# ISU-PAAL/DeepDFA

Hardware: NVIDIA H100
Metric: CFG graphs/sec (train step) (higher is better)
Workload: dtype f32 (GRU GEMMs: bf16x3 split operands, f32 accumulate)

## Files before the change

deepdfa_b200/csrc/abi.cu:

```cuda
#include <stdarg.h>
#include <stdlib.h>
#include <string.h>

#include <atomic>

#include "common.cuh"

namespace ddfa {
static std::atomic<long long> g_launches{0};
void count_launch() { g_launches.fetch_add(1, std::memory_order_relaxed); }

static thread_local char g_err[512] = "";

static thread_local bool g_chain_break = true;
void chain_break() { g_chain_break = true; }
bool chain_take_break() {
  const bool b = g_chain_break;
  g_chain_break = false;
  return b;
}

static std::atomic<int> g_tuning[DDFA_TUNE__COUNT] = {
    {23},
    {15},
    {9},
    {0},
    {2},
    {0},
};
int l2_hints() { return g_tuning[DDFA_TUNE_L2_HINTS].load(std::memory_order_relaxed); }
int pdl_mask() { return g_tuning[DDFA_TUNE_PDL_MASK].load(std::memory_order_relaxed); }
int gather_variant() { return g_tuning[DDFA_TUNE_GATHER_VARIANT].load(std::memory_order_relaxed); }
int gate_bwd_tma() { return g_tuning[DDFA_TUNE_GATE_BWD_TMA].load(std::memory_order_relaxed); }
int gather_src_groups() { return g_tuning[DDFA_TUNE_GATHER_SRC_GROUPS].load(std::memory_order_relaxed); }

void set_error(const char *fmt, ...) {
  va_list ap;
  va_start(ap, fmt);
  vsnprintf(g_err, sizeof(g_err), fmt, ap);
  va_end(ap);
}
}

extern "C" {

int ddfa_abi_version(void) { return DDFA_ABI_VERSION; }

const char *ddfa_last_error(void) { return ddfa::g_err; }

int ddfa_engine_available(int engine) {
  if (engine == DDFA_ENGINE_SIMT) return 1;
  if (engine == DDFA_ENGINE_TCGEN05) return 1;
  return 0;
}

int ddfa_tuning_set(int key, int value) {
  DDFA_REQUIRE(key >= 0 && key < DDFA_TUNE__COUNT, "ddfa_tuning_set: unknown key %d", key);
  DDFA_REQUIRE(key != DDFA_TUNE_FWD_PAIR || value == 0, "ddfa_tuning_set: DDFA_TUNE_FWD_PAIR must be 0 (no CTA-pair forward kernel on sm_90a)");
  ddfa::g_tuning[key].store(value, std::memory_order_relaxed);
  return DDFA_OK;
}
int ddfa_tuning_get(int key) {
  if (key < 0 || key >= DDFA_TUNE__COUNT) return -1;
  return ddfa::g_tuning[key].load(std::memory_order_relaxed);
}

int ddfa_debug_set(int key, int value) {
  switch (key) {
    case 2: {
      int rc = ddfa::gru_tc3_trace_enable(value);
      return rc != DDFA_OK ? rc : ddfa::gru_tc2b_trace_enable(value);
    }
    default: ddfa::set_error("ddfa_debug_set: unknown key %d", key); return DDFA_ERR_INVALID_ARG;
  }
}

int ddfa_debug_read(int key, void *host_out, size_t bytes) {
  DDFA_REQUIRE(host_out != nullptr, "ddfa_debug_read: null output");
  switch (key) {
    case 2: return ddfa::gru_tc2b_trace_read(host_out, bytes);
    case 3: return ddfa::gru_tc3_trace_read(host_out, bytes);
    case 4: {
      DDFA_REQUIRE(bytes >= sizeof(int), "ddfa_debug_read: key 4 needs 4 bytes");
      const int v = ddfa::gather_tma_errors();
      memcpy(host_out, &v, sizeof(int));
      return DDFA_OK;
    }
    default: ddfa::set_error("ddfa_debug_read: unknown key %d", key); return DDFA_ERR_INVALID_ARG;
  }
}

long long ddfa_launch_count(void) { return ddfa::g_launches.load(std::memory_order_relaxed); }

int ddfa_device_supported(void) {
  int dev = 0;
  DDFA_CUDA(cudaGetDevice(&dev));
  int major = 0, minor = 0;
  DDFA_CUDA(cudaDeviceGetAttribute(&major, cudaDevAttrComputeCapabilityMajor, dev));
  DDFA_CUDA(cudaDeviceGetAttribute(&minor, cudaDevAttrComputeCapabilityMinor, dev));
  return (major == 9 && minor == 0) ? 1 : 0;
}

}
```

deepdfa_b200/csrc/common.cuh:

```cuda
#pragma once
#include <cuda_runtime.h>
#include <stdint.h>
#include <stdio.h>

#include "../../include/ddfa_b200.h"

namespace ddfa {

void set_error(const char *fmt, ...);
void count_launch();

inline cudaStream_t as_stream(void *s) { return reinterpret_cast<cudaStream_t>(s); }

#define DDFA_REQUIRE(cond, ...)            \
  do {                                     \
    if (!(cond)) {                         \
      ddfa::set_error(__VA_ARGS__);        \
      return DDFA_ERR_INVALID_ARG;         \
    }                                      \
  } while (0)

#define DDFA_CHECK_LAUNCH(name)                                                        \
  do {                                                                                 \
    cudaError_t e__ = cudaGetLastError();                                              \
    if (e__ != cudaSuccess) {                                                          \
      ddfa::set_error("%s: launch failed: %s", name, cudaGetErrorString(e__));         \
      return DDFA_ERR_CUDA;                                                            \
    }                                                                                  \
    ddfa::count_launch();                                                              \
  } while (0)

#define DDFA_CUDA(call)                                                                \
  do {                                                                                 \
    cudaError_t e__ = (call);                                                          \
    if (e__ != cudaSuccess) {                                                          \
      ddfa::set_error("%s failed: %s", #call, cudaGetErrorString(e__));                \
      return DDFA_ERR_CUDA;                                                            \
    }                                                                                  \
  } while (0)

__device__ __forceinline__ void pdl_launch_dependents() { asm volatile("griddepcontrol.launch_dependents;" ::: "memory"); }
__device__ __forceinline__ void pdl_wait() { asm volatile("griddepcontrol.wait;" ::: "memory"); }
int pdl_mask();
int gather_variant();
int gather_src_groups();
int gate_bwd_tma();
void chain_break();
bool chain_take_break();

template <typename... KArgs, typename... Args>
inline cudaError_t launch_chain_cluster(int which, int cluster_x, void (*kernel)(KArgs...), dim3 grid, dim3 block, size_t smem,
                                        cudaStream_t stream, Args... args) {
  cudaLaunchConfig_t cfg = {};
  cfg.gridDim = grid;
  cfg.blockDim = block;
  cfg.dynamicSmemBytes = smem;
  cfg.stream = stream;
  cudaLaunchAttribute attr[2];
  int n = 0;
  if (cluster_x > 1) {
    attr[n].id = cudaLaunchAttributeClusterDimension;
    attr[n].val.clusterDim.x = (unsigned)cluster_x;
    attr[n].val.clusterDim.y = 1;
    attr[n].val.clusterDim.z = 1;
    ++n;
  }
  const bool brk = chain_take_break();
  if ((pdl_mask() & which) && !brk) {
    attr[n].id = cudaLaunchAttributeProgrammaticStreamSerialization;
    attr[n].val.programmaticStreamSerializationAllowed = 1;
    ++n;
  }
  cfg.attrs = attr;
  cfg.numAttrs = n;
  return cudaLaunchKernelEx(&cfg, kernel, static_cast<KArgs>(args)...);
}
template <typename... KArgs, typename... Args>
inline cudaError_t launch_chain(int which, void (*kernel)(KArgs...), dim3 grid, dim3 block, size_t smem, cudaStream_t stream, Args... args) {
  return launch_chain_cluster(which, 1, kernel, grid, block, smem, stream, args...);
}

int adam_step_inc_launch(int32_t *step_count, cudaStream_t stream);

inline bool aligned16(const void *p) { return (reinterpret_cast<uintptr_t>(p) & 15u) == 0; }

constexpr int kNumSMs = 132;

int sgemm(int ta, int tb, int M, int N, int K, float alpha, const float *A, int lda, const float *B, int ldb,
          float beta, float *C, int ldc, int split_k, cudaStream_t stream);
size_t act_image_bytes(int64_t n);
int act_to_image(const float *x, int32_t N, void *image, cudaStream_t stream);
size_t gru_tc3_packed_bytes();
int gru_tc3_prepare(const float *w_fold, const float *b_fold, const float *b_ih, const float *w_hh, const float *b_hh, void *packed,
                    cudaStream_t stream);
int gru_tc3_step_fwd(const void *s_img, const void *h_img, const float *h, const int32_t *indptr, int32_t N, float *h_out,
                     void *h_out_img, float *save_gates, void *save_gates_packed, const void *packed, cudaStream_t stream);
int gru_tc3_trace_enable(int on);
int gru_tc3_trace_read(void *host, size_t bytes);
int gru_tc2b_trace_enable(int on);
int gru_tc2b_trace_read(void *host, size_t bytes);
size_t gru_tc2_workspace_bytes();
int gru_tc2_prepare(const float *w_fold, const float *b_fold, const float *b_ih, const float *w_hh, const float *b_hh,
                    void *workspace, size_t workspace_bytes, cudaStream_t stream);
int gru_tc2_step_fwd(const void *s_img, const void *h_img, const float *h, const int32_t *indptr, int32_t N, float *h_out,
                     void *h_out_img, float *save_gates, void *save_gates_packed, const void *workspace, size_t workspace_bytes,
                     cudaStream_t stream);
size_t gru_tc2_bwd_workspace_bytes(int32_t N, int32_t slots);
void *gru_tc2_bwd_s_image_scratch(void *workspace, int32_t N);
int gru_tc2_prepare_bwd(const float *w_fold, const float *w_hh, void *workspace, size_t workspace_bytes, cudaStream_t stream);
int gru_tc2_step_bwd(const float *dh_out, const float *ds_in, const int32_t *indptr_t, const int32_t *indices_t, const float *h,
                     const void *h_img_in, const void *s_img, const float *gates, const void *gates_packed, const int32_t *indptr, int32_t N, float *ds, float *dh, float *dw_fold, float *db_fold, float *db_ih,
                     float *dw_hh, float *db_hh, void *workspace, size_t workspace_bytes, int wgrad_mode, cudaStream_t stream);
int gru_tc2_bwd_finish(int32_t N, float *dw_fold, float *dw_hh, void *workspace, size_t workspace_bytes, cudaStream_t stream);
int gru_tc2_bwd_wgrad_batched(const void *const *s_imgs, const void *const *h_imgs, int32_t steps, int32_t N, float *dw_fold,
                              float *dw_hh, void *workspace, size_t workspace_bytes, cudaStream_t stream);

int launch_gather_tma(int variant, const int32_t *indptr, const int32_t *indices, const float *h, int32_t N, float *out, int accumulate,
                      cudaStream_t stream);
int gather_tma_errors();

__device__ __forceinline__ float4 ldg_nc_f4(const float *p) {
  float4 v;
  asm volatile("ld.global.nc.v4.f32 {%0,%1,%2,%3}, [%4];"
               : "=f"(v.x), "=f"(v.y), "=f"(v.z), "=f"(v.w)
               : "l"(p));
  return v;
}

__device__ __forceinline__ float4 ldg_cg_f4(const float *p) { return __ldcg(reinterpret_cast<const float4 *>(p)); }

__device__ __forceinline__ uint64_t l2_policy(int kind) {
  uint64_t p;
  if (kind == 1) asm volatile("createpolicy.fractional.L2::evict_first.b64 %0, 1.0;" : "=l"(p));
  else if (kind == 2) asm volatile("createpolicy.fractional.L2::evict_last.b64 %0, 1.0;" : "=l"(p));
  else asm volatile("createpolicy.fractional.L2::evict_normal.b64 %0, 1.0;" : "=l"(p));
  return p;
}
__device__ __forceinline__ void st_f32_hint(float *p, float v, uint64_t pol) {
  asm volatile("st.global.L2::cache_hint.f32 [%0], %1, %2;" ::"l"(p), "f"(v), "l"(pol) : "memory");
}
__device__ __forceinline__ void st_f4_hint(float *p, const float4 &v, uint64_t pol) {
  asm volatile("st.global.L2::cache_hint.v4.f32 [%0], {%1,%2,%3,%4}, %5;" ::"l"(p), "f"(v.x), "f"(v.y), "f"(v.z), "f"(v.w), "l"(pol) : "memory");
}
__device__ __forceinline__ void st_f2_hint(float *p, const float2 &v, uint64_t pol) {
  asm volatile("st.global.L2::cache_hint.v2.f32 [%0], {%1,%2}, %3;" ::"l"(p), "f"(v.x), "f"(v.y), "l"(pol) : "memory");
}
__device__ __forceinline__ void st_u4_hint(void *p, const uint4 &v, uint64_t pol) {
  asm volatile("st.global.L2::cache_hint.v4.u32 [%0], {%1,%2,%3,%4}, %5;" ::"l"(p), "r"(v.x), "r"(v.y), "r"(v.z), "r"(v.w), "l"(pol) : "memory");
}
__device__ __forceinline__ float4 ldg_cg_f4_hint(const float *p, uint64_t pol) {
  float4 v;
  asm volatile("ld.global.cg.L2::cache_hint.v4.f32 {%0,%1,%2,%3}, [%4], %5;" : "=f"(v.x), "=f"(v.y), "=f"(v.z), "=f"(v.w) : "l"(p), "l"(pol));
  return v;
}
__device__ __forceinline__ float ldg_cg_f32_hint(const float *p, uint64_t pol) {
  float v;
  asm volatile("ld.global.cg.L2::cache_hint.f32 %0, [%1], %2;" : "=f"(v) : "l"(p), "l"(pol));
  return v;
}
__device__ __forceinline__ void st_u32_hint(void *p, uint32_t v, uint64_t pol) {
  asm volatile("st.global.L2::cache_hint.u32 [%0], %1, %2;" ::"l"(p), "r"(v), "l"(pol) : "memory");
}
__device__ __forceinline__ void st_u2_hint(void *p, const uint2 &v, uint64_t pol) {
  asm volatile("st.global.L2::cache_hint.v2.u32 [%0], {%1,%2}, %3;" ::"l"(p), "r"(v.x), "r"(v.y), "l"(pol) : "memory");
}
__device__ __forceinline__ void st_f32_hint_if(bool pred, float *p, float v, uint64_t pol) {
  asm volatile("{\n.reg .pred q;\nsetp.ne.b32 q, %3, 0;\n@q st.global.L2::cache_hint.f32 [%0], %1, %2;\n}" ::"l"(p), "f"(v), "l"(pol), "r"((int)pred) : "memory");
}
__device__ __forceinline__ void st_u32_hint_if(bool pred, void *p, uint32_t v, uint64_t pol) {
  asm volatile("{\n.reg .pred q;\nsetp.ne.b32 q, %3, 0;\n@q st.global.L2::cache_hint.u32 [%0], %1, %2;\n}" ::"l"(p), "r"(v), "l"(pol), "r"((int)pred) : "memory");
}
__device__ __forceinline__ void st_u2_hint_if(bool pred, void *p, const uint2 &v, uint64_t pol) {
  asm volatile("{\n.reg .pred q;\nsetp.ne.b32 q, %4, 0;\n@q st.global.L2::cache_hint.v2.u32 [%0], {%1,%2}, %3;\n}" ::"l"(p), "r"(v.x), "r"(v.y), "l"(pol), "r"((int)pred)
               : "memory");
}
int l2_hints();

__device__ __forceinline__ float warp_sum(float v) {
#pragma unroll
  for (int o = 16; o > 0; o >>= 1) v += __shfl_xor_sync(0xffffffffu, v, o);
  return v;
}
__device__ __forceinline__ float warp_max(float v) {
#pragma unroll
  for (int o = 16; o > 0; o >>= 1) v = fmaxf(v, __shfl_xor_sync(0xffffffffu, v, o));
  return v;
}

__device__ __forceinline__ float sigmoidf_acc(float x) { return 1.0f / (1.0f + expf(-x)); }

__device__ __forceinline__ void f4_add(float4 &a, const float4 &b) {
  a.x += b.x; a.y += b.y; a.z += b.z; a.w += b.w;
}
__device__ __forceinline__ void f4_fma(float4 &a, float s, const float4 &b) {
  a.x = fmaf(s, b.x, a.x); a.y = fmaf(s, b.y, a.y); a.z = fmaf(s, b.z, a.z); a.w = fmaf(s, b.w, a.w);
}
__device__ __forceinline__ float f4_dot(const float4 &a, const float4 &b) {
  return a.x * b.x + a.y * b.y + a.z * b.z + a.w * b.w;
}

}
```

deepdfa_b200/csrc/gru_step.cu:

```cuda
#include "common.cuh"

namespace ddfa {

__global__ void __launch_bounds__(256) gru_gate_fwd_kernel(const float *__restrict__ gi_raw, const float *__restrict__ gh_raw,
                                                           const float *__restrict__ h, const int32_t *__restrict__ indptr,
                                                           const float *__restrict__ b_fold, const float *__restrict__ b_ih,
                                                           const float *__restrict__ b_hh, int32_t N, int32_t D,
                                                           float *__restrict__ h_out, float *__restrict__ gates) {
  const int dq = D >> 2;
  const int64_t t = blockIdx.x * (int64_t)blockDim.x + threadIdx.x;
  if (t >= (int64_t)N * dq) return;
  const int32_t n = (int32_t)(t / dq);
  const int c = (int)(t - (int64_t)n * dq) * 4;
  const float deg = (float)(indptr[n + 1] - indptr[n]);
  const float *gi = gi_raw + (int64_t)n * 3 * D;
  const float *gh = gh_raw + (int64_t)n * 3 * D;
  const float4 hv = *reinterpret_cast<const float4 *>(h + (int64_t)n * D + c);
  float4 g[3][2];
#pragma unroll
  for (int q = 0; q < 3; ++q) {
    const float4 a = *reinterpret_cast<const float4 *>(gi + q * D + c);
    const float4 bf = *reinterpret_cast<const float4 *>(b_fold + q * D + c);
    const float4 bi = *reinterpret_cast<const float4 *>(b_ih + q * D + c);
    g[q][0] = make_float4(fmaf(deg, bf.x, a.x) + bi.x, fmaf(deg, bf.y, a.y) + bi.y, fmaf(deg, bf.z, a.z) + bi.z,
                          fmaf(deg, bf.w, a.w) + bi.w);
    const float4 b = *reinterpret_cast<const float4 *>(gh + q * D + c);
    const float4 bh = *reinterpret_cast<const float4 *>(b_hh + q * D + c);
    g[q][1] = make_float4(b.x + bh.x, b.y + bh.y, b.z + bh.z, b.w + bh.w);
  }
  float4 r, z, nn, o;
#define GATE(f)                                            \
  r.f = sigmoidf_acc(g[0][0].f + g[0][1].f);               \
  z.f = sigmoidf_acc(g[1][0].f + g[1][1].f);               \
  nn.f = tanhf(fmaf(r.f, g[2][1].f, g[2][0].f));           \
  o.f = fmaf(z.f, hv.f - nn.f, nn.f);
  GATE(x) GATE(y) GATE(z) GATE(w)
#undef GATE
  *reinterpret_cast<float4 *>(h_out + (int64_t)n * D + c) = o;
  if (gates) {
    const int64_t plane = (int64_t)N * D, off = (int64_t)n * D + c;
    *reinterpret_cast<float4 *>(gates + off) = r;
    *reinterpret_cast<float4 *>(gates + plane + off) = z;
    *reinterpret_cast<float4 *>(gates + 2 * plane + off) = nn;
    *reinterpret_cast<float4 *>(gates + 3 * plane + off) = g[2][1];
  }
}

constexpr int kGateBwdRows = 128;
__global__ void __launch_bounds__(256) gru_gate_bwd_kernel(const float *__restrict__ dh_out, const float *__restrict__ h,
                                                           const float *__restrict__ gates, const int32_t *__restrict__ indptr,
                                                           int32_t N, int32_t D, float *__restrict__ dgi, float *__restrict__ dgh,
                                                           float *__restrict__ dh_part, float *__restrict__ db_fold,
                                                           float *__restrict__ db_ih, float *__restrict__ db_hh) {
  extern __shared__ float red[];
  const int c = threadIdx.x * 4;
  const int64_t plane = (int64_t)N * D;
  float4 acc[7];
#pragma unroll
  for (int i = 0; i < 7; ++i) acc[i] = make_float4(0.f, 0.f, 0.f, 0.f);
  const int32_t row0 = blockIdx.x * kGateBwdRows;
  const int32_t row1 = min(N, row0 + kGateBwdRows);
  for (int32_t n = row0 + threadIdx.y; n < row1; n += blockDim.y) {
    const int64_t off = (int64_t)n * D + c;
    const float deg = (float)(indptr[n + 1] - indptr[n]);
    const float4 d = *reinterpret_cast<const float4 *>(dh_out + off);
    const float4 hv = *reinterpret_cast<const float4 *>(h + off);
    const float4 r = *reinterpret_cast<const float4 *>(gates + off);
    const float4 z = *reinterpret_cast<const float4 *>(gates + plane + off);
    const float4 nn = *reinterpret_cast<const float4 *>(gates + 2 * plane + off);
    const float4 ghn = *reinterpret_cast<const float4 *>(gates + 3 * plane + off);
    float4 qr, qz, qn, qnr, dhp;
#define BWD(f)                                               \
  {                                                          \
    const float dz = d.f * (hv.f - nn.f);                    \
    const float dn = d.f * (1.f - z.f);                      \
    dhp.f = d.f * z.f;                                       \
    qn.f = dn * (1.f - nn.f * nn.f);                         \
    qz.f = dz * z.f * (1.f - z.f);                           \
    qr.f = qn.f * ghn.f * r.f * (1.f - r.f);                 \
    qnr.f = qn.f * r.f;                                      \
  }
    BWD(x) BWD(y) BWD(z) BWD(w)
#undef BWD
    float *gi = dgi + (int64_t)n * 3 * D + c;
    float *gh = dgh + (int64_t)n * 3 * D + c;
    *reinterpret_cast<float4 *>(gi) = qr;
    *reinterpret_cast<float4 *>(gi + D) = qz;
    *reinterpret_cast<float4 *>(gi + 2 * D) = qn;
    *reinterpret_cast<float4 *>(gh) = qr;
    *reinterpret_cast<float4 *>(gh + D) = qz;
    *reinterpret_cast<float4 *>(gh + 2 * D) = qnr;
    *reinterpret_cast<float4 *>(dh_part + off) = dhp;
    f4_add(acc[0], qr); f4_add(acc[1], qz); f4_add(acc[2], qn); f4_add(acc[3], qnr);
    f4_fma(acc[4], deg, qr); f4_fma(acc[5], deg, qz); f4_fma(acc[6], deg, qn);
  }
#pragma unroll
  for (int i = 0; i < 7; ++i) *reinterpret_cast<float4 *>(&red[((int64_t)threadIdx.y * 7 + i) * D + c]) = acc[i];
  __syncthreads();
  if (threadIdx.y == 0) {
#pragma unroll
    for (int i = 0; i < 7; ++i) {
      float4 sum = acc[i];
      for (int y = 1; y < blockDim.y; ++y) f4_add(sum, *reinterpret_cast<const float4 *>(&red[((int64_t)y * 7 + i) * D + c]));
      acc[i] = sum;
    }
#define RED4(ptr, v) atomicAdd((ptr) + 0, (v).x); atomicAdd((ptr) + 1, (v).y); atomicAdd((ptr) + 2, (v).z); atomicAdd((ptr) + 3, (v).w);
    RED4(db_ih + c, acc[0]) RED4(db_ih + D + c, acc[1]) RED4(db_ih + 2 * D + c, acc[2])
    RED4(db_hh + c, acc[0]) RED4(db_hh + D + c, acc[1]) RED4(db_hh + 2 * D + c, acc[3])
    RED4(db_fold + c, acc[4]) RED4(db_fold + D + c, acc[5]) RED4(db_fold + 2 * D + c, acc[6])
#undef RED4
  }
}

__global__ void fold_bias_kernel(const float *__restrict__ w_ih, const float *__restrict__ b, int32_t D, float *__restrict__ b_fold) {
  const int row = blockIdx.x * (blockDim.x >> 5) + (threadIdx.x >> 5);
  const int lane = threadIdx.x & 31;
  if (row >= 3 * D) return;
  float s = 0.f;
  for (int k = lane; k < D; k += 32) s = fmaf(w_ih[(int64_t)row * D + k], b[k], s);
  s = warp_sum(s);
  if (lane == 0) b_fold[row] = s;
}
__global__ void fold_bias_bwd_outer_kernel(const float *__restrict__ db_fold, const float *__restrict__ b, int32_t D, float *__restrict__ dw_ih) {
  const int64_t t = blockIdx.x * (int64_t)blockDim.x + threadIdx.x;
  if (t >= (int64_t)3 * D * D) return;
  const int j = (int)(t / D), k = (int)(t % D);
  dw_ih[t] = fmaf(db_fold[j], b[k], dw_ih[t]);
}
__global__ void __launch_bounds__(256) fold_bias_bwd_vec_kernel(const float *__restrict__ w_ih, const float *__restrict__ db_fold,
                                                                int32_t D, float *__restrict__ db) {
  __shared__ float red[8][33];
  const int k = blockIdx.x * 32 + threadIdx.x;
  float s = 0.f;
  if (k < D)
    for (int j = threadIdx.y; j < 3 * D; j += 8) s = fmaf(w_ih[(int64_t)j * D + k], db_fold[j], s);
  red[threadIdx.y][threadIdx.x] = s;
  __syncthreads();
  if (threadIdx.y == 0 && k < D) {
    float t = 0.f;
#pragma unroll
    for (int y = 0; y < 8; ++y) t += red[y][threadIdx.x];
    db[k] += t;
  }
}

}

extern "C" {

int ddfa_fold_weights_fwd(const float *w_msg, const float *b_msg, const float *w_ih, int32_t D, float *w_fold,
                          float *b_fold, void *stream_) {
  using namespace ddfa;
  DDFA_REQUIRE(D > 0 && D % 4 == 0, "ddfa_fold_weights_fwd: D=%d must be a positive multiple of 4", D);
  DDFA_REQUIRE(w_msg && b_msg && w_ih && w_fold && b_fold, "ddfa_fold_weights_fwd: NULL pointer");
  cudaStream_t stream = as_stream(stream_);
  int rc = sgemm(0, 0, 3 * D, D, D, 1.f, w_ih, D, w_msg, D, 0.f, w_fold, D, 1, stream);
  if (rc) return rc;
  fold_bias_kernel<<<(3 * D + 7) / 8, 256, 0, stream>>>(w_ih, b_msg, D, b_fold);
  DDFA_CHECK_LAUNCH("fold_bias_kernel");
  return DDFA_OK;
}

int ddfa_fold_weights_bwd(const float *w_msg, const float *b_msg, const float *w_ih, const float *dw_fold,
                          const float *db_fold, int32_t D, float *dw_msg, float *db_msg, float *dw_ih, void *stream_) {
  using namespace ddfa;
  DDFA_REQUIRE(D > 0 && D % 4 == 0, "ddfa_fold_weights_bwd: D=%d must be a positive multiple of 4", D);
  DDFA_REQUIRE(w_msg && b_msg && w_ih && dw_fold && db_fold && dw_msg && db_msg && dw_ih, "ddfa_fold_weights_bwd: NULL pointer");
  cudaStream_t stream = as_stream(stream_);
  int rc = sgemm(0, 1, 3 * D, D, D, 1.f, dw_fold, D, w_msg, D, 1.f, dw_ih, D, 1, stream);
  if (rc) return rc;
  rc = sgemm(1, 0, D, D, 3 * D, 1.f, w_ih, D, dw_fold, D, 1.f, dw_msg, D, 1, stream);
  if (rc) return rc;
  const int64_t tot = (int64_t)3 * D * D;
  fold_bias_bwd_outer_kernel<<<(unsigned)((tot + 255) / 256), 256, 0, stream>>>(db_fold, b_msg, D, dw_ih);
  DDFA_CHECK_LAUNCH("fold_bias_bwd_outer_kernel");
  fold_bias_bwd_vec_kernel<<<(D + 31) / 32, dim3(32, 8), 0, stream>>>(w_ih, db_fold, D, db_msg);
  DDFA_CHECK_LAUNCH("fold_bias_bwd_vec_kernel");
  return DDFA_OK;
}

size_t ddfa_gru_step_workspace_bytes(int32_t N, int32_t D, int engine) {
  if (N < 0 || D <= 0) return 0;
  if (engine == DDFA_ENGINE_TCGEN05) return D == 128 ? ddfa::gru_tc2_workspace_bytes() + 2 * ddfa::act_image_bytes(N) : 16;
  return sizeof(float) * 2 * (size_t)N * 3 * (size_t)D;
}

size_t ddfa_act_image_bytes(int64_t num_nodes) { return num_nodes < 0 ? 0 : ddfa::act_image_bytes(num_nodes); }

int ddfa_act_to_image(const float *x, int32_t N, int32_t D, void *image, void *stream_) {
  using namespace ddfa;
  DDFA_REQUIRE(N >= 0 && D == 128, "ddfa_act_to_image: activation images exist for D == 128 only (N=%d D=%d)", N, D);
  if (N == 0) return DDFA_OK;
  DDFA_REQUIRE(x && image && aligned16(x) && aligned16(image), "ddfa_act_to_image: NULL or unaligned pointer");
  return act_to_image(x, N, image, as_stream(stream_));
}

int ddfa_gru_step_fwd_image(const void *s_image, const void *h_image, const float *h, const int32_t *indptr, int32_t N,
                            int32_t D, float *h_out, void *h_out_image, float *save_gates, const void *workspace,
                            size_t workspace_bytes, void *stream_) {
  using namespace ddfa;
  DDFA_REQUIRE(N >= 0 && D == 128, "ddfa_gru_step_fwd_image: the tcgen05 engine supports D == 128 only (N=%d D=%d)", N, D);
  if (N == 0) return DDFA_OK;
  DDFA_REQUIRE(s_image && h_image && h && indptr && h_out, "ddfa_gru_step_fwd_image: NULL pointer");
  return gru_tc2_step_fwd(s_image, h_image, h, indptr, N, h_out, h_out_image, save_gates, nullptr, workspace, workspace_bytes,
                          as_stream(stream_));
}

size_t ddfa_gru_gates_packed_bytes(int32_t N, int32_t D) { return (N < 0 || D <= 0) ? 0 : (size_t)N * (size_t)D * 8; }

int ddfa_gru_step_fwd_image_v2(const void *s_image, const void *h_image, const float *h, const int32_t *indptr, int32_t N, int32_t D,
                               float *h_out, void *h_out_image, void *save_gates_packed, const void *workspace, size_t workspace_bytes,
                               void *stream_) {
  using namespace ddfa;
  DDFA_REQUIRE(N >= 0 && D == 128, "ddfa_gru_step_fwd_image_v2: the tcgen05 engine supports D == 128 only (N=%d D=%d)", N, D);
  if (N == 0) return DDFA_OK;
  DDFA_REQUIRE(s_image && h_image && indptr, "ddfa_gru_step_fwd_image_v2: NULL pointer");
  DDFA_REQUIRE(h_out || h_out_image, "ddfa_gru_step_fwd_image_v2: neither h_out nor h_out_image given");
  return gru_tc2_step_fwd(s_image, h_image, h, indptr, N, h_out, h_out_image, nullptr, save_gates_packed, workspace, workspace_bytes,
                          as_stream(stream_));
}

static int check_step_args(const char *who, int32_t N, int32_t D, int engine) {
  using namespace ddfa;
  DDFA_REQUIRE(N >= 0 && D > 0 && D % 4 == 0 && D <= 1024, "%s: unsupported shape N=%d D=%d", who, N, D);
  DDFA_REQUIRE(engine == DDFA_ENGINE_SIMT || engine == DDFA_ENGINE_TCGEN05, "%s: unknown engine %d", who, engine);
  if (engine == DDFA_ENGINE_TCGEN05 && D != 128) {
    set_error("%s: the tcgen05 engine supports D == 128 only (got %d); select DDFA_ENGINE_SIMT", who, D);
    return DDFA_ERR_UNSUPPORTED;
  }
  return DDFA_OK;
}

int ddfa_gru_step_prepare(const float *w_fold, const float *b_fold, const float *b_ih, const float *w_hh, const float *b_hh,
                          int32_t D, int engine, void *workspace, size_t workspace_bytes, void *stream_) {
  using namespace ddfa;
  int rc = check_step_args("ddfa_gru_step_prepare", 0, D, engine);
  if (rc) return rc;
  if (engine == DDFA_ENGINE_SIMT) return DDFA_OK;
  DDFA_REQUIRE(w_fold && b_fold && b_ih && w_hh && b_hh, "ddfa_gru_step_prepare: NULL pointer");
  return gru_tc2_prepare(w_fold, b_fold, b_ih, w_hh, b_hh, workspace, workspace_bytes, as_stream(stream_));
}

int ddfa_gru_step_fwd(const float *s, const float *h, const int32_t *indptr, const float *w_fold, const float *b_fold,
                      const float *b_ih, const float *w_hh, const float *b_hh, int32_t N, int32_t D, float *h_out,
                      float *save_gates, void *workspace, size_t workspace_bytes, int engine, void *stream_) {
  using namespace ddfa;
  int rc = check_step_args("ddfa_gru_step_fwd", N, D, engine);
  if (rc) return rc;
  if (N == 0) return DDFA_OK;
  DDFA_REQUIRE(s && h && indptr && w_fold && b_fold && b_ih && w_hh && b_hh && h_out, "ddfa_gru_step_fwd: NULL pointer");
  cudaStream_t stream = as_stream(stream_);
  if (workspace_bytes < ddfa_gru_step_workspace_bytes(N, D, engine) || workspace == nullptr) {
    set_error("ddfa_gru_step_fwd: workspace too small (%zu < %zu)", workspace_bytes, ddfa_gru_step_workspace_bytes(N, D, engine));
    return DDFA_ERR_WORKSPACE;
  }
  if (engine == DDFA_ENGINE_TCGEN05) {
    uint8_t *ws8 = static_cast<uint8_t *>(workspace);
    void *s_img = ws8 + gru_tc2_workspace_bytes();
    void *h_img = ws8 + gru_tc2_workspace_bytes() + act_image_bytes(N);
    rc = act_to_image(s, N, s_img, stream);
    if (rc) return rc;
    rc = act_to_image(h, N, h_img, stream);
    if (rc) return rc;
    return gru_tc2_step_fwd(s_img, h_img, h, indptr, N, h_out, nullptr, save_gates, nullptr, workspace, workspace_bytes, stream);
  }
  float *gi = static_cast<float *>(workspace);
  float *gh = gi + (size_t)N * 3 * D;
  rc = sgemm(0, 1, N, 3 * D, D, 1.f, s, D, w_fold, D, 0.f, gi, 3 * D, 1, stream);
  if (rc) return rc;
  rc = sgemm(0, 1, N, 3 * D, D, 1.f, h, D, w_hh, D, 0.f, gh, 3 * D, 1, stream);
  if (rc) return rc;
  const int64_t tot = (int64_t)N * (D / 4);
  gru_gate_fwd_kernel<<<(unsigned)((tot + 255) / 256), 256, 0, stream>>>(gi, gh, h, indptr, b_fold, b_ih, b_hh, N, D, h_out, save_gates);
  DDFA_CHECK_LAUNCH("gru_gate_fwd_kernel");
  return DDFA_OK;
}

size_t ddfa_gru_step_bwd_workspace_bytes(int32_t N, int32_t D, int engine) {
  if (N < 0 || D <= 0) return 0;
  return ddfa_gru_step_bwd_workspace_bytes_steps(N, D, engine, 1);
}

size_t ddfa_gru_step_bwd_workspace_bytes_steps(int32_t N, int32_t D, int engine, int32_t steps) {
  if (N < 0 || D <= 0) return 0;
  if (engine == DDFA_ENGINE_TCGEN05) return D == 128 ? ddfa::gru_tc2_bwd_workspace_bytes(N, steps) : 16;
  return sizeof(float) * 2 * (size_t)N * 3 * (size_t)D;
}

int ddfa_gru_bwd_wgrad_batched(const void *const *s_images, const void *const *h_images, int32_t steps, int32_t N, int32_t D,
                               float *dw_fold, float *dw_hh, void *workspace, size_t workspace_bytes, void *stream_) {
  using namespace ddfa;
  DDFA_REQUIRE(N >= 0 && D == 128, "ddfa_gru_bwd_wgrad_batched: the tcgen05 engine supports D == 128 only (N=%d D=%d)", N, D);
  DDFA_REQUIRE(s_images && h_images && dw_fold && dw_hh, "ddfa_gru_bwd_wgrad_batched: NULL pointer");
  if (N == 0) return DDFA_OK;
  return gru_tc2_bwd_wgrad_batched(s_images, h_images, steps, N, dw_fold, dw_hh, workspace, workspace_bytes, as_stream(stream_));
}

int ddfa_gru_step_bwd_image(const float *dh_out, const float *ds_prev, const int32_t *indptr_t, const int32_t *indices_t,
                            const float *h, const void *h_image, const void *s_image, const float *gates,
                            const int32_t *indptr, int32_t N, int32_t D, float *ds, float *dh, float *dw_fold, float *db_fold,
                            float *db_ih, float *dw_hh, float *db_hh, void *workspace, size_t workspace_bytes, int wgrad_mode,
                            void *stream_) {
  using namespace ddfa;
  DDFA_REQUIRE(N >= 0 && D == 128, "ddfa_gru_step_bwd_image: the tcgen05 engine supports D == 128 only (N=%d D=%d)", N, D);
  DDFA_REQUIRE((wgrad_mode >= 0 && wgrad_mode <= 2) || (wgrad_mode >= 16 && wgrad_mode < 32),
               "ddfa_gru_step_bwd_image: wgrad_mode must be 0, 1, 2 or DDFA_WGRAD_KEEP(slot < 16) (got %d)", wgrad_mode);
  if (N == 0) return DDFA_OK;
  DDFA_REQUIRE(dh_out && h && s_image && gates && indptr && ds && dh && dw_fold && db_fold && db_ih && dw_hh && db_hh,
               "ddfa_gru_step_bwd_image: NULL pointer");
  DDFA_REQUIRE(dh != dh_out, "ddfa_gru_step_bwd_image: dh must not alias dh_out");
  DDFA_REQUIRE(ds_prev == nullptr || (indptr_t && indices_t), "ddfa_gru_step_bwd_image: ds_prev given without the transposed CSR");
  DDFA_REQUIRE(ds_prev == nullptr || ds_prev != ds, "ddfa_gru_step_bwd_image: ds must not alias ds_prev");
  return gru_tc2_step_bwd(dh_out, ds_prev, indptr_t, indices_t, h, h_image, s_image, gates, nullptr, indptr, N, ds, dh, dw_fold, db_fold, db_ih, dw_hh, db_hh, workspace,
                          workspace_bytes, wgrad_mode, as_stream(stream_));
}

int ddfa_gru_step_bwd_image_v2(const float *dh_out, const float *ds_prev, const int32_t *indptr_t, const int32_t *indices_t,
                               const float *h, const void *h_image, const void *s_image, const void *gates_packed,
                               const int32_t *indptr, int32_t N, int32_t D, float *ds, float *dh, float *dw_fold, float *db_fold,
                               float *db_ih, float *dw_hh, float *db_hh, void *workspace, size_t workspace_bytes, int wgrad_mode,
                               void *stream_) {
  using namespace ddfa;
  DDFA_REQUIRE(N >= 0 && D == 128, "ddfa_gru_step_bwd_image_v2: the tcgen05 engine supports D == 128 only (N=%d D=%d)", N, D);
  DDFA_REQUIRE((wgrad_mode >= 0 && wgrad_mode <= 2) || (wgrad_mode >= 16 && wgrad_mode < 32),
               "ddfa_gru_step_bwd_image_v2: wgrad_mode must be 0, 1, 2 or DDFA_WGRAD_KEEP(slot < 16) (got %d)", wgrad_mode);
  if (N == 0) return DDFA_OK;
  DDFA_REQUIRE(dh_out && h_image && s_image && gates_packed && indptr && ds && dh && dw_fold && db_fold && db_ih && dw_hh && db_hh,
               "ddfa_gru_step_bwd_image_v2: NULL pointer");
  DDFA_REQUIRE(dh != dh_out, "ddfa_gru_step_bwd_image_v2: dh must not alias dh_out");
  DDFA_REQUIRE(ds_prev == nullptr || (indptr_t && indices_t), "ddfa_gru_step_bwd_image_v2: ds_prev given without the transposed CSR");
  DDFA_REQUIRE(ds_prev == nullptr || ds_prev != ds, "ddfa_gru_step_bwd_image_v2: ds must not alias ds_prev");
  return gru_tc2_step_bwd(dh_out, ds_prev, indptr_t, indices_t, h, h_image, s_image, nullptr, gates_packed, indptr, N, ds, dh, dw_fold, db_fold,
                          db_ih, dw_hh, db_hh, workspace, workspace_bytes, wgrad_mode, as_stream(stream_));
}

int ddfa_gru_step_bwd_finish(int32_t N, int32_t D, float *dw_fold, float *dw_hh, void *workspace, size_t workspace_bytes,
                             void *stream_) {
  using namespace ddfa;
  DDFA_REQUIRE(N >= 0 && D == 128 && dw_fold && dw_hh, "ddfa_gru_step_bwd_finish: bad arguments (N=%d D=%d)", N, D);
  if (N == 0) return DDFA_OK;
  return gru_tc2_bwd_finish(N, dw_fold, dw_hh, workspace, workspace_bytes, as_stream(stream_));
}

int ddfa_gru_step_prepare_bwd(const float *w_fold, const float *w_hh, int32_t D, int engine, void *workspace,
                              size_t workspace_bytes, void *stream_) {
  using namespace ddfa;
  int rc = check_step_args("ddfa_gru_step_prepare_bwd", 0, D, engine);
  if (rc) return rc;
  if (engine == DDFA_ENGINE_SIMT) return DDFA_OK;
  DDFA_REQUIRE(w_fold && w_hh, "ddfa_gru_step_prepare_bwd: NULL pointer");
  return gru_tc2_prepare_bwd(w_fold, w_hh, workspace, workspace_bytes, as_stream(stream_));
}

int ddfa_gru_step_bwd(const float *dh_out, const float *h, const float *s, const float *gates, const int32_t *indptr,
                      const float *w_fold, const float *w_hh, int32_t N, int32_t D, float *ds, float *dh,
                      float *dw_fold, float *db_fold, float *db_ih, float *dw_hh, float *db_hh, void *workspace,
                      size_t workspace_bytes, int engine, void *stream_) {
  using namespace ddfa;
  int rc = check_step_args("ddfa_gru_step_bwd", N, D, engine);
  if (rc) return rc;
  if (N == 0) return DDFA_OK;
  DDFA_REQUIRE(dh_out && h && s && gates && indptr && w_fold && w_hh && ds && dh && dw_fold && db_fold && db_ih && dw_hh && db_hh,
               "ddfa_gru_step_bwd: NULL pointer");
  DDFA_REQUIRE(dh != dh_out, "ddfa_gru_step_bwd: dh must not alias dh_out");
  cudaStream_t stream = as_stream(stream_);
  const size_t need = ddfa_gru_step_bwd_workspace_bytes(N, D, engine);
  if (workspace_bytes < need || workspace == nullptr) {
    set_error("ddfa_gru_step_bwd: workspace too small (%zu < %zu)", workspace_bytes, need);
    return DDFA_ERR_WORKSPACE;
  }
  if (engine == DDFA_ENGINE_TCGEN05) {
    void *s_img = gru_tc2_bwd_s_image_scratch(workspace, N);
    rc = act_to_image(s, N, s_img, stream);
    if (rc) return rc;
    return gru_tc2_step_bwd(dh_out, nullptr, nullptr, nullptr, h, nullptr, s_img, gates, nullptr, indptr, N, ds, dh, dw_fold, db_fold, db_ih, dw_hh, db_hh,
                            workspace, workspace_bytes, 0, stream);
  }
  float *dgi = static_cast<float *>(workspace);
  float *dgh = dgi + (size_t)N * 3 * D;
  dim3 block(D / 4, 256 / (D / 4) > 0 ? 256 / (D / 4) : 1);
  const size_t smem = sizeof(float) * block.y * 7 * D;
  gru_gate_bwd_kernel<<<(N + kGateBwdRows - 1) / kGateBwdRows, block, smem, stream>>>(dh_out, h, gates, indptr, N, D, dgi, dgh, dh,
                                                                                     db_fold, db_ih, db_hh);
  DDFA_CHECK_LAUNCH("gru_gate_bwd_kernel");
  rc = sgemm(0, 0, N, D, 3 * D, 1.f, dgi, 3 * D, w_fold, D, 0.f, ds, D, 1, stream);
  if (rc) return rc;
  rc = sgemm(0, 0, N, D, 3 * D, 1.f, dgh, 3 * D, w_hh, D, 1.f, dh, D, 1, stream);
  if (rc) return rc;
  const int tiles = ((3 * D + 127) / 128) * ((D + 127) / 128);
  int split = (2 * kNumSMs + tiles - 1) / tiles;
  const int k_tiles = (N + 15) / 16;
  if (split > k_tiles / 8) split = k_tiles / 8 > 0 ? k_tiles / 8 : 1;
  rc = sgemm(1, 0, 3 * D, D, N, 1.f, dgi, 3 * D, s, D, 1.f, dw_fold, D, split, stream);
  if (rc) return rc;
  rc = sgemm(1, 0, 3 * D, D, N, 1.f, dgh, 3 * D, h, D, 1.f, dw_hh, D, split, stream);
  return rc;
}

}
```

deepdfa_b200/csrc/gru_tc_bwd.cu:

```cuda
#include <cuda_fp16.h>

#include "tc_common.cuh"

namespace ddfa {
namespace tc2b {
using namespace tcc;

constexpr int kThreads = 320, kEpiWarps = 8;

constexpr int kGbWarps = 8;
struct GbRow {
  float4 d, hv, rr, zz, nn, gh;
  float deg;
  int tb, te;
};
__device__ __forceinline__ float4 bf16x4_to_f4(const uint2 &p) {
  return make_float4(__uint_as_float(p.x << 16), __uint_as_float(p.x & 0xffff0000u), __uint_as_float(p.y << 16), __uint_as_float(p.y & 0xffff0000u));
}
__device__ __forceinline__ void gb_load(GbRow &x, const float *__restrict__ dh_out, const float *__restrict__ h,
                                        const uint8_t *__restrict__ h_img_src, const float *__restrict__ gates,
                                        const uint4 *__restrict__ gates_packed, const int32_t *__restrict__ indptr,
                                        const int32_t *__restrict__ indptr_t, size_t plane, int64_t node, int col, bool ok,
                                        uint64_t pol_saved, uint64_t pol_dh) {
  x.tb = x.te = 0;
  if (ok) {
    if (indptr_t) { x.tb = __ldcg(indptr_t + node); x.te = __ldcg(indptr_t + node + 1); }
    const size_t off = (size_t)node * kD + col;
    x.d = ldg_cg_f4_hint(dh_out + off, pol_dh);
    uint2 hh = make_uint2(0u, 0u), hl = hh;
    uint4 g0 = make_uint4(0u, 0u, 0u, 0u), g1 = g0;
    if (h) x.hv = ldg_cg_f4_hint(h + off, pol_saved);
    else {
      hh = __ldcg(reinterpret_cast<const uint2 *>(h_img_src + image_offset(node, col, 0)));
      hl = __ldcg(reinterpret_cast<const uint2 *>(h_img_src + image_offset(node, col, 1)));
    }
    if (gates) {
      x.rr = ldg_cg_f4_hint(gates + off, pol_saved);
      x.zz = ldg_cg_f4_hint(gates + plane + off, pol_saved);
      x.nn = ldg_cg_f4_hint(gates + 2 * plane + off, pol_saved);
      x.gh = ldg_cg_f4_hint(gates + 3 * plane + off, pol_saved);
    } else {
      g0 = __ldcg(gates_packed + (off >> 1));
      g1 = __ldcg(gates_packed + (off >> 1) + 1);
    }
    x.deg = (float)(__ldcg(indptr + node + 1) - __ldcg(indptr + node));
    if (!h) {
      const float4 a = bf16x4_to_f4(hh), b = bf16x4_to_f4(hl);
      x.hv = make_float4(a.x + b.x, a.y + b.y, a.z + b.z, a.w + b.w);
    }
    if (!gates) {
      unpack_gates(make_uint2(g0.x, g0.y), x.rr.x, x.zz.x, x.nn.x, x.gh.x);
      unpack_gates(make_uint2(g0.z, g0.w), x.rr.y, x.zz.y, x.nn.y, x.gh.y);
      unpack_gates(make_uint2(g1.x, g1.y), x.rr.z, x.zz.z, x.nn.z, x.gh.z);
      unpack_gates(make_uint2(g1.z, g1.w), x.rr.w, x.zz.w, x.nn.w, x.gh.w);
    }
  }
}

__global__ void __launch_bounds__(32 * kGbWarps, 2) gate_bwd_image_kernel(const float *__restrict__ dh_out, const float *__restrict__ h,
                                                                          const uint8_t *__restrict__ h_img_src,
                                                                          const float *__restrict__ gates, const uint4 *__restrict__ gates_packed,
                                                                          const int32_t *__restrict__ indptr,
                                                                          const float *__restrict__ ds_in, const int32_t *__restrict__ indptr_t,
                                                                          const int32_t *__restrict__ indices_t,
                                                                          int32_t N, uint8_t *__restrict__ q_img, size_t img_stride,
                                                                          uint8_t *__restrict__ h_img, float *__restrict__ dhz,
                                                                          float *__restrict__ db_fold,
                                                                          float *__restrict__ db_ih, float *__restrict__ db_hh, int hints) {
  __shared__ float red[kGbWarps][7 * kD];
  const int lane = threadIdx.x & 31, warp = threadIdx.x >> 5;
  const int col = lane * 4;
  pdl_launch_dependents();
  pdl_wait();
  const uint64_t pol_saved = l2_policy((hints & 2) ? 1 : 0), pol_tmp = l2_policy((hints & 4) ? 2 : 0), pol_dh = l2_policy((hints & 8) ? 1 : 0);
  const size_t plane = (size_t)N * kD;
  float4 sum[7];
#pragma unroll
  for (int i = 0; i < 7; ++i) sum[i] = make_float4(0.f, 0.f, 0.f, 0.f);
  const int64_t Npad = ((int64_t)N + kTileM - 1) / kTileM * kTileM;
  const int64_t stride = (int64_t)gridDim.x * kGbWarps;

  auto finish = [&](const GbRow &x, int64_t node, bool ok) {
    float4 qr = make_float4(0.f, 0.f, 0.f, 0.f), qz = qr, qn = qr, qnr = qr, hv = qr;
    if (ok) {
      hv = x.hv;
      st_f4_hint(dhz + (size_t)node * kD + col, make_float4(x.d.x * x.zz.x, x.d.y * x.zz.y, x.d.z * x.zz.z, x.d.w * x.zz.w), pol_tmp);
#define BWDQ(f)                                                      \
  {                                                                  \
    const float dz_ = x.d.f * (x.hv.f - x.nn.f);                     \
    const float dn_ = x.d.f * (1.f - x.zz.f);                        \
    qn.f = dn_ * (1.f - x.nn.f * x.nn.f);                            \
    qz.f = dz_ * x.zz.f * (1.f - x.zz.f);                            \
    qr.f = qn.f * x.gh.f * x.rr.f * (1.f - x.rr.f);                  \
    qnr.f = qn.f * x.rr.f;                                           \
  }
      BWDQ(x) BWDQ(y) BWDQ(z) BWDQ(w)
#undef BWDQ
      f4_add(sum[0], qr); f4_add(sum[1], qz); f4_add(sum[2], qn); f4_add(sum[3], qnr);
      f4_fma(sum[4], x.deg, qr); f4_fma(sum[5], x.deg, qz); f4_fma(sum[6], x.deg, qn);
    }
    const size_t o_hi = image_offset(node, col, 0), o_lo = image_offset(node, col, 1);
    uint2 ph, pl;
    split4(qr, ph, pl);  *reinterpret_cast<uint2 *>(q_img + 0 * img_stride + o_hi) = ph; *reinterpret_cast<uint2 *>(q_img + 0 * img_stride + o_lo) = pl;
    split4(qz, ph, pl);  *reinterpret_cast<uint2 *>(q_img + 1 * img_stride + o_hi) = ph; *reinterpret_cast<uint2 *>(q_img + 1 * img_stride + o_lo) = pl;
    split4(qn, ph, pl);  *reinterpret_cast<uint2 *>(q_img + 2 * img_stride + o_hi) = ph; *reinterpret_cast<uint2 *>(q_img + 2 * img_stride + o_lo) = pl;
    split4(qnr, ph, pl); *reinterpret_cast<uint2 *>(q_img + 3 * img_stride + o_hi) = ph; *reinterpret_cast<uint2 *>(q_img + 3 * img_stride + o_lo) = pl;
    if (h_img) {
      split4(hv, ph, pl); *reinterpret_cast<uint2 *>(h_img + o_hi) = ph; *reinterpret_cast<uint2 *>(h_img + o_lo) = pl;
    }
  };

  for (int64_t node = (int64_t)blockIdx.x * kGbWarps + warp; node < Npad; node += 2 * stride) {
    const int64_t node2 = node + stride;
    GbRow a, b;
    const bool ok_a = node < N, ok_b = node2 < N;
    gb_load(a, dh_out, h, h_img_src, gates, gates_packed, indptr, indptr_t, plane, node, col, ok_a, pol_saved, pol_dh);
    gb_load(b, dh_out, h, h_img_src, gates, gates_packed, indptr, indptr_t, plane, node2, col, ok_b, pol_saved, pol_dh);
    if (indptr_t) {
      int ia[4], ib[4];
#pragma unroll
      for (int k = 0; k < 4; ++k) {
        ia[k] = (a.tb + k < a.te) ? __ldcg(indices_t + a.tb + k) : -1;
        ib[k] = (b.tb + k < b.te) ? __ldcg(indices_t + b.tb + k) : -1;
      }
      float4 va[4], vb[4];
#pragma unroll
      for (int k = 0; k < 4; ++k) {
        va[k] = ia[k] >= 0 ? ldg_cg_f4(ds_in + (size_t)ia[k] * kD + col) : make_float4(0.f, 0.f, 0.f, 0.f);
        vb[k] = ib[k] >= 0 ? ldg_cg_f4(ds_in + (size_t)ib[k] * kD + col) : make_float4(0.f, 0.f, 0.f, 0.f);
      }
#pragma unroll
      for (int k = 0; k < 4; ++k) { f4_add(a.d, va[k]); f4_add(b.d, vb[k]); }
      for (int j = a.tb + 4; j < a.te; ++j) f4_add(a.d, ldg_cg_f4(ds_in + (size_t)__ldcg(indices_t + j) * kD + col));
      for (int j = b.tb + 4; j < b.te; ++j) f4_add(b.d, ldg_cg_f4(ds_in + (size_t)__ldcg(indices_t + j) * kD + col));
    }
    finish(a, node, ok_a);
    if (node2 < Npad) finish(b, node2, ok_b);
  }
#pragma unroll
  for (int i = 0; i < 7; ++i) *reinterpret_cast<float4 *>(&red[warp][i * kD + col]) = sum[i];
  __syncthreads();
  for (int i = threadIdx.x; i < 7 * kD; i += 32 * kGbWarps) {
    float v_ = 0.f;
#pragma unroll
    for (int w = 0; w < kGbWarps; ++w) v_ += red[w][i];
    const int which = i >> 7, c_ = i & 127;
    if (which == 0) { atomicAdd(db_ih + c_, v_); atomicAdd(db_hh + c_, v_); }
    else if (which == 1) { atomicAdd(db_ih + kD + c_, v_); atomicAdd(db_hh + kD + c_, v_); }
    else if (which == 2) atomicAdd(db_ih + 2 * kD + c_, v_);
    else if (which == 3) atomicAdd(db_hh + 2 * kD + c_, v_);
    else atomicAdd(db_fold + (which - 4) * kD + c_, v_);
  }
}

constexpr int kGtRows = 32, kGtStages = 3, kGtConsumers = 16, kGtPre = 2;
constexpr int kGtOffD = 0, kGtOffG = kGtRows * kD * 4, kGtOffH = kGtOffG + kGtRows * kD * 8;
constexpr int kGtStageBytes = kGtOffH + kGtRows * kD * 4;
constexpr int kGtOffBar = kGtStages * kGtStageBytes;
constexpr int kGtSmem = kGtOffBar + 2 * kGtStages * 8 + 16;
constexpr int kGtThreads = 32 * kGtConsumers;

template <bool HF32, bool CSRP>
__global__ void __launch_bounds__(kGtThreads, 1) gate_bwd_tma_kernel(const float *__restrict__ dh_out, const float *__restrict__ h,
                                                                     const uint8_t *__restrict__ h_img_src, const uint2 *__restrict__ gates_packed,
                                                                     const int32_t *__restrict__ indptr, const float *__restrict__ ds_in,
                                                                     const int32_t *__restrict__ indptr_t, const int32_t *__restrict__ indices_t,
                                                                     int32_t N, uint8_t *__restrict__ q_img, size_t img_stride,
                                                                     float *__restrict__ dhz, float *__restrict__ db_fold, float *__restrict__ db_ih,
                                                                     float *__restrict__ db_hh, int hints) {
  extern __shared__ __align__(1024) uint8_t smem[];
  const uint32_t sbase = smem_u32(smem);
  const uint32_t bar0 = sbase + kGtOffBar;
  auto full = [&](int i) { return bar0 + 8u * i; };
  auto empty = [&](int i) { return bar0 + 8u * (kGtStages + i); };
  const int lane = threadIdx.x & 31, warp = threadIdx.x >> 5;
  const int64_t Npad = ((int64_t)N + kTileM - 1) / kTileM * kTileM;
  const int num_blocks = (int)(Npad / kGtRows);
  const int my_blocks = (num_blocks > (int)blockIdx.x) ? (num_blocks - 1 - (int)blockIdx.x) / (int)gridDim.x + 1 : 0;
  if (threadIdx.x == 0) {
    for (int i = 0; i < kGtStages; ++i) { mbar_init(full(i), 1); mbar_init(empty(i), kGtConsumers); }
    mbar_fence_init();
  }
  __syncthreads();
  pdl_launch_dependents();
  pdl_wait();
  float4 sum[7];
#pragma unroll
  for (int i = 0; i < 7; ++i) sum[i] = make_float4(0.f, 0.f, 0.f, 0.f);

  auto fill = [&](int k) {
    const uint64_t pol_saved = l2_policy((hints & 2) ? 1 : 0), pol_dh = l2_policy((hints & 8) ? 1 : 0);
    const int stage = k % kGtStages;
    const int64_t r0 = (int64_t)(blockIdx.x + (int64_t)k * gridDim.x) * kGtRows;
    const int valid = (int)max((int64_t)0, min((int64_t)kGtRows, (int64_t)N - r0));
    const uint32_t dst = sbase + stage * kGtStageBytes;
    const uint32_t bytes = (uint32_t)valid * (kD * 4 + kD * 8) + (HF32 ? (uint32_t)valid * kD * 4 : (uint32_t)kGtRows * kD * 4);
    mbar_arrive_expect_tx(full(stage), bytes);
    if (valid > 0) {
      bulk_g2s_hint(dst + kGtOffD, dh_out + r0 * kD, (uint32_t)valid * kD * 4, full(stage), pol_dh);
      bulk_g2s_hint(dst + kGtOffG, gates_packed + r0 * kD, (uint32_t)valid * kD * 8, full(stage), pol_saved);
    }
    if (HF32) {
      if (valid > 0) bulk_g2s_hint(dst + kGtOffH, h + r0 * kD, (uint32_t)valid * kD * 4, full(stage), pol_saved);
    } else {
      const uint8_t *tile = h_img_src + (size_t)(r0 >> 7) * kImageTileBytes + (size_t)(r0 & 127) * 128;
#pragma unroll
      for (int ch = 0; ch < 4; ++ch) bulk_g2s_hint(dst + kGtOffH + ch * (kGtRows * 128), tile + (size_t)ch * kChunkBytes, kGtRows * 128, full(stage), pol_saved);
    }
  };
  if (warp == 0 && elect_one())
    for (int k = 0; k < kGtStages && k < my_blocks; ++k) fill(k);
  __syncwarp();
  {
    const int col = lane * 4;
    const uint64_t pol_tmp = l2_policy((hints & 4) ? 2 : 0);
    static_assert(kGtPre == 2, "lane slots below assume two prefetched neighbours per row");
    auto load_scalars = [&](int kk) -> int {
      int v = 0;
      if (kk < my_blocks && lane < 8) {
        const int64_t nd = (int64_t)(blockIdx.x + (int64_t)kk * gridDim.x) * kGtRows + warp + 16 * ((lane >> 1) & 1);
        const int32_t *base = lane < 4 ? indptr : indptr_t;
        if (nd < N && base) v = __ldcg(base + nd + (lane & 1));
      }
      return v;
    };
    auto load_ids = [&](int sc) -> int {
      const int r_ = (lane >> 1) & 1, q_ = lane & 1;
      const int tb_ = __shfl_sync(0xffffffffu, sc, 4 + 2 * r_), te_ = __shfl_sync(0xffffffffu, sc, 5 + 2 * r_);
      int v = -1;
      if (lane >= 8 && lane < 12 && tb_ + q_ < te_) v = __ldcg(indices_t + tb_ + q_);
      return v;
    };
    int sc_cur = 0, sc_next = 0, id_cur = -1;
    if constexpr (CSRP) {
      sc_cur = load_scalars(0); sc_next = load_scalars(1);
      id_cur = load_ids(sc_cur);
    }
    for (int k = 0; k < my_blocks; ++k) {
      const int stage = k % kGtStages, use = k / kGtStages;
      const int64_t r0 = (int64_t)(blockIdx.x + (int64_t)k * gridDim.x) * kGtRows;
      int64_t node[2];
      bool ok[2];
      int tb[2], te[2], ip0[2], ip1[2];
      int id[2][kGtPre];
      if constexpr (CSRP) {
        const int sc_next2 = load_scalars(k + 2);
        const int id_next = load_ids(sc_next);
#pragma unroll
        for (int r = 0; r < 2; ++r) {
          node[r] = r0 + warp + 16 * r;
          ok[r] = node[r] < N;
          ip0[r] = __shfl_sync(0xffffffffu, sc_cur, 2 * r); ip1[r] = __shfl_sync(0xffffffffu, sc_cur, 2 * r + 1);
          tb[r] = __shfl_sync(0xffffffffu, sc_cur, 4 + 2 * r); te[r] = __shfl_sync(0xffffffffu, sc_cur, 5 + 2 * r);
#pragma unroll
          for (int q = 0; q < kGtPre; ++q) id[r][q] = __shfl_sync(0xffffffffu, id_cur, 8 + 2 * r + q);
        }
        sc_cur = sc_next; sc_next = sc_next2; id_cur = id_next;
      } else {
#pragma unroll
        for (int r = 0; r < 2; ++r) {
          node[r] = r0 + warp + 16 * r;
          ok[r] = node[r] < N;
          tb[r] = te[r] = ip0[r] = ip1[r] = 0;
          if (ok[r]) {
            ip0[r] = __ldcg(indptr + node[r]); ip1[r] = __ldcg(indptr + node[r] + 1);
            if (indptr_t) { tb[r] = __ldcg(indptr_t + node[r]); te[r] = __ldcg(indptr_t + node[r] + 1); }
          }
        }
#pragma unroll
        for (int r = 0; r < 2; ++r)
#pragma unroll
          for (int q = 0; q < kGtPre; ++q) id[r][q] = (tb[r] + q < te[r]) ? __ldcg(indices_t + tb[r] + q) : -1;
      }
      float4 gv[2][kGtPre];
#pragma unroll
      for (int r = 0; r < 2; ++r)
#pragma unroll
        for (int q = 0; q < kGtPre; ++q) gv[r][q] = id[r][q] >= 0 ? ldg_cg_f4(ds_in + (size_t)id[r][q] * kD + col) : make_float4(0.f, 0.f, 0.f, 0.f);
      mbar_wait(full(stage), use & 1);
      const uint8_t *st = smem + stage * kGtStageBytes;
#pragma unroll
      for (int r = 0; r < 2; ++r) {
        const int row = warp + 16 * r;
        float4 d = make_float4(0.f, 0.f, 0.f, 0.f), hv = d, rr = d, zz = d, nn = d, gh = d;
        if (ok[r]) {
          d = *reinterpret_cast<const float4 *>(st + kGtOffD + row * (kD * 4) + col * 4);
          const uint4 g0 = *reinterpret_cast<const uint4 *>(st + kGtOffG + row * (kD * 8) + col * 8);
          const uint4 g1 = *reinterpret_cast<const uint4 *>(st + kGtOffG + row * (kD * 8) + col * 8 + 16);
          unpack_gates(make_uint2(g0.x, g0.y), rr.x, zz.x, nn.x, gh.x);
          unpack_gates(make_uint2(g0.z, g0.w), rr.y, zz.y, nn.y, gh.y);
          unpack_gates(make_uint2(g1.x, g1.y), rr.z, zz.z, nn.z, gh.z);
          unpack_gates(make_uint2(g1.z, g1.w), rr.w, zz.w, nn.w, gh.w);
          if (HF32) {
            hv = *reinterpret_cast<const float4 *>(st + kGtOffH + row * (kD * 4) + col * 4);
          } else {
            const uint32_t off = (uint32_t)((col >> 6) * (kGtRows * 128) + row * 128 + (((((col & 63) >> 3) ^ (row & 7)) & 7) << 4) + (col & 7) * 2);
            const uint2 hh = *reinterpret_cast<const uint2 *>(st + kGtOffH + off);
            const uint2 hl = *reinterpret_cast<const uint2 *>(st + kGtOffH + 2 * (kGtRows * 128) + off);
            const float4 a = bf16x4_to_f4(hh), b = bf16x4_to_f4(hl);
            hv = make_float4(a.x + b.x, a.y + b.y, a.z + b.z, a.w + b.w);
          }
#pragma unroll
          for (int q = 0; q < kGtPre; ++q) f4_add(d, gv[r][q]);
          for (int j = tb[r] + kGtPre; j < te[r]; ++j) f4_add(d, ldg_cg_f4(ds_in + (size_t)__ldcg(indices_t + j) * kD + col));
        }
        float4 qr = make_float4(0.f, 0.f, 0.f, 0.f), qz = qr, qn = qr, qnr = qr;
        if (ok[r]) {
          const float deg = (float)(ip1[r] - ip0[r]);
          st_f4_hint(dhz + (size_t)node[r] * kD + col, make_float4(d.x * zz.x, d.y * zz.y, d.z * zz.z, d.w * zz.w), pol_tmp);
#define BWDQ2(f)                                         \
  {                                                      \
    const float dz_ = d.f * (hv.f - nn.f);               \
    const float dn_ = d.f * (1.f - zz.f);                \
    qn.f = dn_ * (1.f - nn.f * nn.f);                    \
    qz.f = dz_ * zz.f * (1.f - zz.f);                    \
    qr.f = qn.f * gh.f * rr.f * (1.f - rr.f);            \
    qnr.f = qn.f * rr.f;                                 \
  }
          BWDQ2(x) BWDQ2(y) BWDQ2(z) BWDQ2(w)
#undef BWDQ2
          f4_add(sum[0], qr); f4_add(sum[1], qz); f4_add(sum[2], qn); f4_add(sum[3], qnr);
          f4_fma(sum[4], deg, qr); f4_fma(sum[5], deg, qz); f4_fma(sum[6], deg, qn);
        }
        if (node[r] < Npad) {
          const size_t o_hi = image_offset(node[r], col, 0), o_lo = image_offset(node[r], col, 1);
          uint2 ph, pl;
          split4(qr, ph, pl);  *reinterpret_cast<uint2 *>(q_img + 0 * img_stride + o_hi) = ph; *reinterpret_cast<uint2 *>(q_img + 0 * img_stride + o_lo) = pl;
          split4(qz, ph, pl);  *reinterpret_cast<uint2 *>(q_img + 1 * img_stride + o_hi) = ph; *reinterpret_cast<uint2 *>(q_img + 1 * img_stride + o_lo) = pl;
          split4(qn, ph, pl);  *reinterpret_cast<uint2 *>(q_img + 2 * img_stride + o_hi) = ph; *reinterpret_cast<uint2 *>(q_img + 2 * img_stride + o_lo) = pl;
          split4(qnr, ph, pl); *reinterpret_cast<uint2 *>(q_img + 3 * img_stride + o_hi) = ph; *reinterpret_cast<uint2 *>(q_img + 3 * img_stride + o_lo) = pl;
        }
      }
      __syncwarp();
      if (lane == 0) mbar_arrive(empty(stage));
      if (warp == 0 && k + kGtStages < my_blocks) {
        if (elect_one()) {
          mbar_wait(empty(stage), use & 1);
          fill(k + kGtStages);
        }
        __syncwarp();
      }
    }
  }
  __syncthreads();
  float *red = reinterpret_cast<float *>(smem);
  {
#pragma unroll
    for (int i = 0; i < 7; ++i) *reinterpret_cast<float4 *>(&red[(warp * 7 + i) * kD + lane * 4]) = sum[i];
  }
  __syncthreads();
  for (int i = threadIdx.x; i < 7 * kD; i += kGtThreads) {
    float v_ = 0.f;
#pragma unroll
    for (int w = 0; w < kGtConsumers; ++w) v_ += red[(w * 7) * kD + i];
    const int which = i >> 7, c_ = i & 127;
    if (which == 0) { atomicAdd(db_ih + c_, v_); atomicAdd(db_hh + c_, v_); }
    else if (which == 1) { atomicAdd(db_ih + kD + c_, v_); atomicAdd(db_hh + kD + c_, v_); }
    else if (which == 2) atomicAdd(db_ih + 2 * kD + c_, v_);
    else if (which == 3) atomicAdd(db_hh + 2 * kD + c_, v_);
    else atomicAdd(db_fold + (which - 4) * kD + c_, v_);
  }
}

constexpr int kD3Stages = 2;
constexpr int kD3StageBytes = kImageTileBytes;
constexpr int kD3WChunkBytes = 64 * 128;
constexpr int kD3WBytes = 12 * kD3WChunkBytes;
constexpr int kD3OffStage = kD3WBytes;
constexpr int kD3OffBar = kD3OffStage + kD3Stages * kD3StageBytes;
constexpr int kD3SmemAlloc = kD3OffBar + (2 * kD3Stages + 1) * 8 + 1024;
constexpr int kD3Threads = 32 * kEpiWarps + 32;
constexpr size_t kD3PackedBytes = (size_t)4 * kD3WBytes;
static_assert(kD3SmemAlloc <= 232448, "shared memory budget");

__global__ void dgrad3_pack_kernel(const float *__restrict__ w_fold, const float *__restrict__ w_hh, uint8_t *__restrict__ packed) {
  const int idx = blockIdx.x * blockDim.x + threadIdx.x;
  if (idx >= 4 * 3 * 64 * 16) return;
  const int u = idx % 16, n = (idx / 16) % 64, g = (idx / (16 * 64)) % 3, rh = idx / (16 * 64 * 3);
  const int role = rh >> 1, half = rh & 1, kb = u >> 3;
  const float *W = role == 0 ? w_fold : w_hh;
  float x[8];
#pragma unroll
  for (int i = 0; i < 8; ++i) x[i] = W[(size_t)(g * kD + u * 8 + i) * kD + half * 64 + n];
  uint4 ph, pl;
  split8(x, ph, pl);
  uint8_t *base = packed + (size_t)rh * kD3WBytes + sw128_offset(n, (u & 7) * 8);
  *reinterpret_cast<uint4 *>(base + ((g * 2 + 0) * 2 + kb) * kD3WChunkBytes) = ph;
  *reinterpret_cast<uint4 *>(base + ((g * 2 + 1) * 2 + kb) * kD3WChunkBytes) = pl;
}

__global__ void __launch_bounds__(kD3Threads, 1) dgrad3_kernel(const uint8_t *__restrict__ q_img, size_t img_stride,
                                                               const float *__restrict__ dhz, const uint8_t *__restrict__ packed3,
                                                               int32_t N, float *__restrict__ ds, float *__restrict__ dh, int hints) {
  extern __shared__ uint8_t smem_raw[];
  uint8_t *smem = reinterpret_cast<uint8_t *>((reinterpret_cast<uintptr_t>(smem_raw) + 1023) & ~(uintptr_t)1023);
  const uint32_t sbase = smem_u32(smem);
  const uint32_t bar0 = sbase + kD3OffBar;
  auto full = [&](int i) { return bar0 + 8u * i; };
  auto empty = [&](int i) { return bar0 + 8u * (kD3Stages + i); };
  const uint32_t w_full = bar0 + 8u * (2 * kD3Stages);
  const int tron = (g_trace_on == 1);

  const int warp = threadIdx.x >> 5, lane = threadIdx.x & 31;
  const int rh = blockIdx.x & 3, role = rh >> 1, half = rh & 1;
  const int group = blockIdx.x >> 2, num_groups = gridDim.x >> 2;
  const int num_tiles = (N + kTileM - 1) / kTileM;
  const int my_tiles = (num_tiles > group) ? (num_tiles - 1 - group) / num_groups + 1 : 0;

  if (threadIdx.x == 0) {
    for (int i = 0; i < kD3Stages; ++i) { mbar_init(full(i), 1); mbar_init(empty(i), kEpiWarps); }
    mbar_init(w_full, 1);
    mbar_fence_init();
  }
  __syncthreads();
  if (threadIdx.x == 0) trace_stamp(tron, 0, 0);
  pdl_launch_dependents();

  if (warp == kEpiWarps) {
    if (my_tiles > 0 && elect_one()) {
      mbar_arrive_expect_tx(w_full, kD3WBytes);
      bulk_g2s(sbase, packed3 + (size_t)rh * kD3WBytes, kD3WBytes, w_full);
      pdl_wait();
      const uint64_t pol_q = l2_policy((hints & 64) ? 1 : 0);
      int cc = 0;
      for (int k = 0; k < my_tiles; ++k) {
        const int tile = num_tiles - 1 - (group + k * num_groups);
        for (int g = 0; g < 3; ++g, ++cc) {
          const int m = g < 2 ? g : (role == 0 ? 2 : 3);
          const int stage = cc % kD3Stages, use = cc / kD3Stages;
          if (use > 0) mbar_wait_bounded(empty(stage), (use - 1) & 1);
          mbar_arrive_expect_tx(full(stage), kD3StageBytes);
          bulk_g2s_hint(sbase + kD3OffStage + stage * kD3StageBytes, q_img + (size_t)m * img_stride + (size_t)tile * kImageTileBytes,
                        kD3StageBytes, full(stage), pol_q);
          if (g != 1) trace_stamp(tron, k, g == 0 ? 1 : 2);
        }
      }
    }
    return;
  }

  pdl_wait();
  if (my_tiles == 0) return;
  const int wg = warp >> 2;
  const int row0 = wg * 64 + (warp & 3) * 16 + (lane >> 2);
  const int col0 = half * 64 + 2 * (lane & 3);
  float *out = role == 0 ? ds : dh;
  const uint64_t pol_tmp = l2_policy((hints & 4) ? 2 : 0);
  const uint64_t pol_dhz = l2_policy((hints & 8) ? 1 : 0);
  mbar_wait_bounded(w_full, 0);
  const bool tr = (warp == 0 && lane == 0);
  int cc = 0, pending = -1;
  for (int k = 0; k < my_tiles; ++k) {
    const int tile = num_tiles - 1 - (group + k * num_groups);
    float acc[32];
    if (tr) { trace_stamp(tron, k, 7); trace_stamp(tron, k, 3); }
    for (int g = 0; g < 3; ++g, ++cc) {
      const int stage = cc % kD3Stages, use = cc / kD3Stages;
      mbar_wait_bounded(full(stage), use & 1);
      if (tr && g != 1) trace_stamp(tron, k, g == 0 ? 4 : 5);
      wgmma_fence();
      const uint32_t a0 = sbase + kD3OffStage + stage * kD3StageBytes + wg * 8192;
      const uint32_t w0 = sbase + g * 4 * kD3WChunkBytes;
#pragma unroll
      for (int kb = 0; kb < 2; ++kb) {
#pragma unroll
        for (int k4 = 0; k4 < 4; ++k4) {
          const uint64_t a_hi = gmma_desc(a0 + kb * kChunkBytes + k4 * 32), a_lo = gmma_desc(a0 + (2 + kb) * kChunkBytes + k4 * 32);
          const uint64_t b_hi = gmma_desc(w0 + kb * kD3WChunkBytes + k4 * 32), b_lo = gmma_desc(w0 + (2 + kb) * kD3WChunkBytes + k4 * 32);
          wgmma_n64<0, 0>(acc, a_hi, b_hi, (g == 0 && kb == 0 && k4 == 0) ? 0u : 1u);
          wgmma_n64<0, 0>(acc, a_hi, b_lo, 1u);
          wgmma_n64<0, 0>(acc, a_lo, b_hi, 1u);
        }
      }
      wgmma_commit();
      wgmma_wait<1>();
      __syncwarp();
      if (pending >= 0 && lane == 0) mbar_arrive(empty(pending));
      pending = stage;
    }
    float2 dv[2][8];
#pragma unroll
    for (int hh = 0; hh < 2; ++hh) {
      const int64_t node = (int64_t)tile * kTileM + row0 + 8 * hh;
#pragma unroll
      for (int j = 0; j < 8; ++j) {
        dv[hh][j] = make_float2(0.f, 0.f);
        if (role == 1 && node < N) {
          const float *p = dhz + node * kD + col0 + 8 * j;
          dv[hh][j] = make_float2(ldg_cg_f32_hint(p, pol_dhz), ldg_cg_f32_hint(p + 1, pol_dhz));
        }
      }
    }
    wgmma_wait<0>();
    wgmma_fence_regs(acc);
    if (tr) { trace_stamp(tron, k, 6); trace_stamp(tron, k, 8); }
    __syncwarp();
    if (lane == 0) mbar_arrive(empty(pending));
    pending = -1;
    if (tr) trace_stamp(tron, k, 9);
#pragma unroll
    for (int hh = 0; hh < 2; ++hh) {
      const int64_t node = (int64_t)tile * kTileM + row0 + 8 * hh;
      if (node < N) {
#pragma unroll
        for (int j = 0; j < 8; ++j)
          st_f2_hint(out + node * kD + col0 + 8 * j, make_float2(acc[4 * j + 2 * hh] + dv[hh][j].x, acc[4 * j + 2 * hh + 1] + dv[hh][j].y), pol_tmp);
      }
    }
    if (tr) trace_stamp(tron, k, 10);
  }
}

constexpr int kWgSlotBytes = kImageTileBytes;
constexpr int kWgSlots = 3;
constexpr int kWgOffBar = kWgSlots * kWgSlotBytes;
constexpr int kWgSmemAlloc = kWgOffBar + 2 * kWgSlots * 8 + 1024;
constexpr int kWgThreads = 32 * kEpiWarps + 32;
constexpr size_t kWgPartialFloats = (size_t)3 * kD * kD;
constexpr int kWgMaxSteps = 16;
struct WgBatch {
  const uint8_t *s_img[kWgMaxSteps];
  const uint8_t *h_img[kWgMaxSteps];
  int32_t steps;
};
__global__ void __launch_bounds__(kWgThreads, 1) wgrad_kernel(const uint8_t *__restrict__ q_img, size_t img_stride, size_t step_stride,
                                                              const __grid_constant__ WgBatch batch,
                                                              int32_t N, float *__restrict__ partial, int first, int hints) {
  extern __shared__ uint8_t smem_raw[];
  uint8_t *smem = reinterpret_cast<uint8_t *>((reinterpret_cast<uintptr_t>(smem_raw) + 1023) & ~(uintptr_t)1023);
  const uint32_t sbase = smem_u32(smem);
  const uint32_t bar0 = sbase + kWgOffBar;
  auto full = [&](int i) { return bar0 + 8u * i; };
  auto empty = [&](int i) { return bar0 + 8u * (kWgSlots + i); };

  const int warp = threadIdx.x >> 5, lane = threadIdx.x & 31;
  const int role = blockIdx.y / 3, g = blockIdx.y % 3;
  const int qm = g < 2 ? g : (role == 0 ? 2 : 3);
  const int num_tiles = (N + kTileM - 1) / kTileM;
  const int all_tiles = num_tiles * batch.steps;
  const int my_tiles = (all_tiles > (int)blockIdx.x) ? (all_tiles - 1 - (int)blockIdx.x) / (int)gridDim.x + 1 : 0;

  if (threadIdx.x == 0) {
    for (int i = 0; i < kWgSlots; ++i) { mbar_init(full(i), 1); mbar_init(empty(i), kEpiWarps); }
    mbar_fence_init();
  }
  __syncthreads();
  const int tron = (g_trace_on == 2) && blockIdx.y == 0;
  if (threadIdx.x == 0) trace_stamp(tron, 0, 0);

  if (warp == kEpiWarps) {
    if (elect_one()) {
      const uint64_t pol_wg = l2_policy((hints & 32) ? 1 : 0);
      for (int i = 0; i < my_tiles; ++i) {
        const int idx = (int)blockIdx.x + i * (int)gridDim.x;
        const int t = idx / num_tiles, tile = idx - t * num_tiles;
        for (int w = 0; w < 2; ++w) {
          const int cc = 2 * i + w, slot = cc % kWgSlots, use = cc / kWgSlots;
          if (use > 0) mbar_wait_bounded(empty(slot), (use - 1) & 1);
          const uint8_t *src = w == 0 ? (role == 0 ? batch.s_img[t] : batch.h_img[t]) : q_img + (size_t)t * step_stride + (size_t)qm * img_stride;
          mbar_arrive_expect_tx(full(slot), kWgSlotBytes);
          bulk_g2s_hint(sbase + slot * kWgSlotBytes, src + (size_t)tile * kImageTileBytes, kWgSlotBytes, full(slot), pol_wg);
          trace_stamp(tron, i, 1 + w);
        }
      }
    }
    return;
  }

  const int wg = warp >> 2;
  float acc[64], sum[64];
#pragma unroll
  for (int i = 0; i < 64; ++i) acc[i] = sum[i] = 0.f;
  for (int i = 0; i < my_tiles; ++i) {
    const int cb = 2 * i, ca = 2 * i + 1;
    mbar_wait_bounded(full(cb % kWgSlots), (cb / kWgSlots) & 1);
    if (warp == 0 && lane == 0) trace_stamp(tron, i, 3);
    mbar_wait_bounded(full(ca % kWgSlots), (ca / kWgSlots) & 1);
    if (warp == 0 && lane == 0) { trace_stamp(tron, i, 4); trace_stamp(tron, i, 5); }
    const uint32_t b0 = sbase + (cb % kWgSlots) * kWgSlotBytes;
    const uint32_t a0 = sbase + (ca % kWgSlots) * kWgSlotBytes + wg * kChunkBytes;
    constexpr uint32_t vs = 2 * kChunkBytes;
    wgmma_fence();
#pragma unroll
    for (int k16 = 0; k16 < kTileM / 16; ++k16) {
      const uint32_t koff = (uint32_t)k16 * 2048u;
      const uint64_t a_hi = gmma_desc(a0 + koff, kChunkBytes), a_lo = gmma_desc(a0 + vs + koff, kChunkBytes);
      const uint64_t b_hi = gmma_desc(b0 + koff, kChunkBytes), b_lo = gmma_desc(b0 + vs + koff, kChunkBytes);
      wgmma_n128<1, 1>(acc, a_hi, b_hi, k16 == 0 ? 0u : 1u);
      wgmma_n128<1, 1>(acc, a_lo, b_hi, 1u);
      wgmma_n128<1, 1>(acc, a_hi, b_lo, 1u);
    }
    wgmma_commit();
    if (warp == 0 && lane == 0) trace_stamp(tron, i, 6);
    wgmma_wait<0>();
    wgmma_fence_regs(acc);
    __syncwarp();
    if (lane == 0) { mbar_arrive(empty(cb % kWgSlots)); mbar_arrive(empty(ca % kWgSlots)); }
#pragma unroll
    for (int j = 0; j < 64; ++j) sum[j] += acc[j];
  }
  if (warp == 0 && lane == 0) trace_stamp(tron, 0, 8);
  float *dst = partial + ((size_t)role * gridDim.x + blockIdx.x) * kWgPartialFloats;
  const int row0 = g * kD + wg * 64 + (warp & 3) * 16 + (lane >> 2);
#pragma unroll
  for (int hh = 0; hh < 2; ++hh) {
    float *rowp = dst + (size_t)(row0 + 8 * hh) * kD + 2 * (lane & 3);
#pragma unroll
    for (int j = 0; j < 16; ++j) {
      float2 v = make_float2(sum[4 * j + 2 * hh], sum[4 * j + 2 * hh + 1]);
      if (!first) {
        const float2 o = *reinterpret_cast<const float2 *>(rowp + 8 * j);
        v.x += o.x;
        v.y += o.y;
      }
      *reinterpret_cast<float2 *>(rowp + 8 * j) = v;
    }
  }
  if (warp == 0 && lane == 0) trace_stamp(tron, 0, 10);
}

__global__ void __launch_bounds__(256) wgrad_reduce_kernel(const float *__restrict__ partial, int ctas, float *__restrict__ dw_fold,
                                                           float *__restrict__ dw_hh) {
  const int i = blockIdx.x * blockDim.x + threadIdx.x;
  const int role = blockIdx.y;
  if (i >= (int)(kWgPartialFloats / 4)) return;
  const float4 *src = reinterpret_cast<const float4 *>(partial + (size_t)role * ctas * kWgPartialFloats) + i;
  float4 s = make_float4(0.f, 0.f, 0.f, 0.f);
  for (int c = 0; c < ctas; ++c) f4_add(s, src[(size_t)c * (kWgPartialFloats / 4)]);
  float4 *dst = reinterpret_cast<float4 *>(role == 0 ? dw_fold : dw_hh) + i;
  float4 d = *dst;
  f4_add(d, s);
  *dst = d;
}

}

constexpr int kWgCtas = kNumSMs / 6;
static size_t wg_partial_bytes() { return (size_t)2 * kWgCtas * tc2b::kWgPartialFloats * sizeof(float); }
int gru_tc2b_trace_enable(int on) {
  DDFA_CUDA(cudaMemcpyToSymbol(tcc::g_trace_on, &on, sizeof(int)));
  return DDFA_OK;
}
int gru_tc2b_trace_read(void *host, size_t bytes) {
  if (bytes > tcc::kTraceWords * sizeof(long long)) bytes = tcc::kTraceWords * sizeof(long long);
  DDFA_CUDA(cudaMemcpyFromSymbol(host, tcc::g_trace, bytes));
  return DDFA_OK;
}
static constexpr size_t kPackedTotal = tc2b::kD3PackedBytes;
static size_t bwd_fixed_bytes(int32_t N) { return kPackedTotal + 3 * tcc::image_bytes(N) + wg_partial_bytes(); }
void *gru_tc2_bwd_s_image_scratch(void *workspace, int32_t N) { return static_cast<uint8_t *>(workspace) + kPackedTotal + 2 * tcc::image_bytes(N); }
size_t gru_tc2_bwd_workspace_bytes(int32_t N, int32_t slots) {
  return bwd_fixed_bytes(N) + (size_t)(slots < 1 ? 1 : slots) * 4 * tcc::image_bytes(N);
}


int gru_tc2_prepare_bwd(const float *w_fold, const float *w_hh, void *workspace, size_t workspace_bytes, cudaStream_t stream) {
  if (workspace == nullptr || workspace_bytes < kPackedTotal) {
    set_error("tcgen05 engine (bwd): workspace too small");
    return DDFA_ERR_WORKSPACE;
  }
  const int total = 4 * 3 * 64 * 16;
  tc2b::dgrad3_pack_kernel<<<(total + 127) / 128, 128, 0, stream>>>(w_fold, w_hh, static_cast<uint8_t *>(workspace));
  DDFA_CHECK_LAUNCH("tc2b::dgrad3_pack_kernel");
  chain_break();
  return DDFA_OK;
}

int gru_tc2_bwd_finish(int32_t N, float *dw_fold, float *dw_hh, void *workspace, size_t workspace_bytes, cudaStream_t stream) {
  if (workspace == nullptr || workspace_bytes < gru_tc2_bwd_workspace_bytes(N, 1)) {
    set_error("tcgen05 engine (bwd finish): workspace too small");
    return DDFA_ERR_WORKSPACE;
  }
  float *partial = reinterpret_cast<float *>(static_cast<uint8_t *>(workspace) + kPackedTotal + 3 * tcc::image_bytes(N));
  const int n4 = (int)(tc2b::kWgPartialFloats / 4);
  tc2b::wgrad_reduce_kernel<<<dim3((n4 + 255) / 256, 2), 256, 0, stream>>>(partial, kWgCtas, dw_fold, dw_hh);
  DDFA_CHECK_LAUNCH("tc2b::wgrad_reduce_kernel");
  return DDFA_OK;
}

int gru_tc2_step_bwd(const float *dh_out, const float *ds_in, const int32_t *indptr_t, const int32_t *indices_t, const float *h,
                     const void *h_img_in, const void *s_img, const float *gates, const void *gates_packed, const int32_t *indptr, int32_t N, float *ds, float *dh, float *dw_fold, float *db_fold, float *db_ih,
                     float *dw_hh, float *db_hh, void *workspace, size_t workspace_bytes, int wgrad_mode, cudaStream_t stream) {
  if (h == nullptr && h_img_in == nullptr) {
    set_error("tcgen05 engine (bwd): neither the fp32 h nor its activation image given");
    return DDFA_ERR_INVALID_ARG;
  }
  const int q_slot = wgrad_mode >= 16 ? wgrad_mode - 16 : 0;
  if (workspace == nullptr || workspace_bytes < gru_tc2_bwd_workspace_bytes(N, q_slot + 1)) {
    set_error("tcgen05 engine (bwd): workspace too small (%zu < %zu)", workspace_bytes, gru_tc2_bwd_workspace_bytes(N, q_slot + 1));
    return DDFA_ERR_WORKSPACE;
  }
  uint8_t *packed = static_cast<uint8_t *>(workspace);
  const size_t img = tcc::image_bytes(N);
  uint8_t *h_img_ws = packed + kPackedTotal;
  float *dhz = reinterpret_cast<float *>(h_img_ws + img);
  float *partial = reinterpret_cast<float *>(h_img_ws + 3 * img);
  uint8_t *q_img = packed + bwd_fixed_bytes(N) + (size_t)q_slot * 4 * img;
  const uint8_t *h_img = h_img_in ? static_cast<const uint8_t *>(h_img_in) : h_img_ws;
  const int64_t rows = ((int64_t)N + tcc::kTileM - 1) / tcc::kTileM * tcc::kTileM;
  unsigned gb_grid = 1;
  {
    const int64_t want = (rows + tc2b::kGbWarps - 1) / tc2b::kGbWarps;
    gb_grid = (unsigned)(want < 2 * kNumSMs ? want : 2 * kNumSMs);
  }
  if (gates_packed && gate_bwd_tma()) {
    const int blocks32 = (int)(rows / tc2b::kGtRows);
    const int grid = blocks32 < kNumSMs ? blocks32 : kNumSMs;
    const bool csrp = gate_bwd_tma() >= 2;
#define DDFA_GT_LAUNCH(HF32, CSRP)                                                                                                             \
  do {                                                                                                                                         \
    DDFA_CUDA(cudaFuncSetAttribute(tc2b::gate_bwd_tma_kernel<HF32, CSRP>, cudaFuncAttributeMaxDynamicSharedMemorySize, tc2b::kGtSmem));        \
    DDFA_CUDA(launch_chain(4, tc2b::gate_bwd_tma_kernel<HF32, CSRP>, dim3(grid), dim3(tc2b::kGtThreads), tc2b::kGtSmem, stream, dh_out, h,     \
                           static_cast<const uint8_t *>(h_img_in), static_cast<const uint2 *>(gates_packed), indptr, ds_in,                    \
                           ds_in ? indptr_t : nullptr, indices_t, N, q_img, img, dhz, db_fold, db_ih, db_hh, l2_hints()));                    \
  } while (0)
    if (h) { if (csrp) DDFA_GT_LAUNCH(true, true); else DDFA_GT_LAUNCH(true, false); }
    else   { if (csrp) DDFA_GT_LAUNCH(false, true); else DDFA_GT_LAUNCH(false, false); }
#undef DDFA_GT_LAUNCH
  } else
  DDFA_CUDA(launch_chain(4, tc2b::gate_bwd_image_kernel, dim3(gb_grid), dim3(32 * tc2b::kGbWarps), 0, stream, dh_out, h,
                         static_cast<const uint8_t *>(h_img_in), gates, static_cast<const uint4 *>(gates_packed), indptr, ds_in,
                         ds_in ? indptr_t : nullptr, indices_t, N, q_img, img, h_img_in ? nullptr : h_img_ws, dhz, db_fold, db_ih, db_hh,
                         l2_hints()));
  DDFA_CHECK_LAUNCH("tc2b::gate_bwd_image_kernel");
  DDFA_CUDA(cudaFuncSetAttribute(tc2b::wgrad_kernel, cudaFuncAttributeMaxDynamicSharedMemorySize, tc2b::kWgSmemAlloc));
  const int tiles = (N + tcc::kTileM - 1) / tcc::kTileM;
  {
    DDFA_CUDA(cudaFuncSetAttribute(tc2b::dgrad3_kernel, cudaFuncAttributeMaxDynamicSharedMemorySize, tc2b::kD3SmemAlloc));
    int groups = kNumSMs / 4;
    if (groups > tiles) groups = tiles;
    DDFA_CUDA(launch_chain(8, tc2b::dgrad3_kernel, dim3(groups * 4), dim3(tc2b::kD3Threads), tc2b::kD3SmemAlloc, stream, q_img, img, dhz,
                           static_cast<const uint8_t *>(packed), N, ds, dh, l2_hints()));
    DDFA_CHECK_LAUNCH("tc2b::dgrad3_kernel");
  }
  if (wgrad_mode >= 16) return DDFA_OK;
  tc2b::WgBatch one = {};
  one.s_img[0] = static_cast<const uint8_t *>(s_img);
  one.h_img[0] = h_img;
  one.steps = 1;
  tc2b::wgrad_kernel<<<dim3(kWgCtas, 6), tc2b::kWgThreads, tc2b::kWgSmemAlloc, stream>>>(q_img, img, 0, one, N, partial, wgrad_mode == 2 ? 0 : 1, 0);
  DDFA_CHECK_LAUNCH("tc2b::wgrad_kernel");
  if (wgrad_mode == 0) return gru_tc2_bwd_finish(N, dw_fold, dw_hh, workspace, workspace_bytes, stream);
  return DDFA_OK;
}

int gru_tc2_bwd_wgrad_batched(const void *const *s_imgs, const void *const *h_imgs, int32_t steps, int32_t N, float *dw_fold,
                              float *dw_hh, void *workspace, size_t workspace_bytes, cudaStream_t stream) {
  if (steps < 1 || steps > tc2b::kWgMaxSteps) {
    set_error("tcgen05 engine (batched wgrad): 1 <= steps <= %d required (got %d)", tc2b::kWgMaxSteps, steps);
    return DDFA_ERR_INVALID_ARG;
  }
  if (workspace == nullptr || workspace_bytes < gru_tc2_bwd_workspace_bytes(N, steps)) {
    set_error("tcgen05 engine (batched wgrad): workspace too small (%zu < %zu)", workspace_bytes, gru_tc2_bwd_workspace_bytes(N, steps));
    return DDFA_ERR_WORKSPACE;
  }
  uint8_t *packed = static_cast<uint8_t *>(workspace);
  const size_t img = tcc::image_bytes(N);
  float *partial = reinterpret_cast<float *>(packed + kPackedTotal + 3 * img);
  const uint8_t *q_img = packed + bwd_fixed_bytes(N);
  tc2b::WgBatch b = {};
  for (int t = 0; t < steps; ++t) {
    if (!s_imgs[t] || !h_imgs[t]) {
      set_error("tcgen05 engine (batched wgrad): NULL image pointer for step %d", t);
      return DDFA_ERR_INVALID_ARG;
    }
    b.s_img[t] = static_cast<const uint8_t *>(s_imgs[t]);
    b.h_img[t] = static_cast<const uint8_t *>(h_imgs[t]);
  }
  b.steps = steps;
  DDFA_CUDA(cudaFuncSetAttribute(tc2b::wgrad_kernel, cudaFuncAttributeMaxDynamicSharedMemorySize, tc2b::kWgSmemAlloc));
  tc2b::wgrad_kernel<<<dim3(kWgCtas, 6), tc2b::kWgThreads, tc2b::kWgSmemAlloc, stream>>>(q_img, img, 4 * img, b, N, partial, 1, l2_hints());
  DDFA_CHECK_LAUNCH("tc2b::wgrad_kernel");
  return gru_tc2_bwd_finish(N, dw_fold, dw_hh, workspace, workspace_bytes, stream);
}

}
```

Measured before the change: 89660.

## Fuse gate backward and dgrad into one clustered persistent kernel

Replaces the separate TMA gate-backward kernel and the dgrad3 kernel with one 4-CTA-cluster kernel. Each cluster computes the gate gradients for its tile, writes the q images, and then runs the dgrad GEMM on them, so the dhz intermediate, one launch and the inter-kernel dependency go away. The grid size comes from an occupancy query for clusters. This adds cluster barriers, proxy fences and more complex synchronisation, and it may limit parallelism during the gate phase.

```diff
diff --git a/deepdfa_b200/csrc/abi.cu b/deepdfa_b200/csrc/abi.cu
--- a/deepdfa_b200/csrc/abi.cu
+++ b/deepdfa_b200/csrc/abi.cu
@@ -86,6 +86,14 @@
       memcpy(host_out, &v, sizeof(int));
       return DDFA_OK;
     }
+    case 5: {
+      DDFA_REQUIRE(bytes >= sizeof(int), "ddfa_debug_read: key 5 needs 4 bytes");
+      int v = 0;
+      const int rc = ddfa::gru_tc2b_fused_max_clusters(&v);
+      if (rc != DDFA_OK) return rc;
+      memcpy(host_out, &v, sizeof(int));
+      return DDFA_OK;
+    }
     default: ddfa::set_error("ddfa_debug_read: unknown key %d", key); return DDFA_ERR_INVALID_ARG;
   }
 }
diff --git a/deepdfa_b200/csrc/common.cuh b/deepdfa_b200/csrc/common.cuh
--- a/deepdfa_b200/csrc/common.cuh
+++ b/deepdfa_b200/csrc/common.cuh
@@ -99,6 +99,7 @@
 int gru_tc3_trace_read(void *host, size_t bytes);
 int gru_tc2b_trace_enable(int on);
 int gru_tc2b_trace_read(void *host, size_t bytes);
+int gru_tc2b_fused_max_clusters(int *out);
 size_t gru_tc2_workspace_bytes();
 int gru_tc2_prepare(const float *w_fold, const float *b_fold, const float *b_ih, const float *w_hh, const float *b_hh,
                     void *workspace, size_t workspace_bytes, cudaStream_t stream);
diff --git a/deepdfa_b200/csrc/gru_step.cu b/deepdfa_b200/csrc/gru_step.cu
--- a/deepdfa_b200/csrc/gru_step.cu
+++ b/deepdfa_b200/csrc/gru_step.cu
@@ -330,6 +330,7 @@
   DDFA_REQUIRE(dh != dh_out, "ddfa_gru_step_bwd_image_v2: dh must not alias dh_out");
   DDFA_REQUIRE(ds_prev == nullptr || (indptr_t && indices_t), "ddfa_gru_step_bwd_image_v2: ds_prev given without the transposed CSR");
   DDFA_REQUIRE(ds_prev == nullptr || ds_prev != ds, "ddfa_gru_step_bwd_image_v2: ds must not alias ds_prev");
+  DDFA_REQUIRE(ds_prev == nullptr || ds_prev != dh, "ddfa_gru_step_bwd_image_v2: dh must not alias ds_prev");
   return gru_tc2_step_bwd(dh_out, ds_prev, indptr_t, indices_t, h, h_image, s_image, nullptr, gates_packed, indptr, N, ds, dh, dw_fold, db_fold,
                           db_ih, dw_hh, db_hh, workspace, workspace_bytes, wgrad_mode, as_stream(stream_));
 }
diff --git a/deepdfa_b200/csrc/gru_tc_bwd.cu b/deepdfa_b200/csrc/gru_tc_bwd.cu
--- a/deepdfa_b200/csrc/gru_tc_bwd.cu
+++ b/deepdfa_b200/csrc/gru_tc_bwd.cu
@@ -1,4 +1,6 @@
 #include <cuda_fp16.h>
+
+#include <atomic>
 
 #include "tc_common.cuh"
 
@@ -144,215 +146,6 @@
     float v_ = 0.f;
 #pragma unroll
     for (int w = 0; w < kGbWarps; ++w) v_ += red[w][i];
-    const int which = i >> 7, c_ = i & 127;
-    if (which == 0) { atomicAdd(db_ih + c_, v_); atomicAdd(db_hh + c_, v_); }
-    else if (which == 1) { atomicAdd(db_ih + kD + c_, v_); atomicAdd(db_hh + kD + c_, v_); }
-    else if (which == 2) atomicAdd(db_ih + 2 * kD + c_, v_);
-    else if (which == 3) atomicAdd(db_hh + 2 * kD + c_, v_);
-    else atomicAdd(db_fold + (which - 4) * kD + c_, v_);
-  }
-}
-
-constexpr int kGtRows = 32, kGtStages = 3, kGtConsumers = 16, kGtPre = 2;
-constexpr int kGtOffD = 0, kGtOffG = kGtRows * kD * 4, kGtOffH = kGtOffG + kGtRows * kD * 8;
-constexpr int kGtStageBytes = kGtOffH + kGtRows * kD * 4;
-constexpr int kGtOffBar = kGtStages * kGtStageBytes;
-constexpr int kGtSmem = kGtOffBar + 2 * kGtStages * 8 + 16;
-constexpr int kGtThreads = 32 * kGtConsumers;
-
-template <bool HF32, bool CSRP>
-__global__ void __launch_bounds__(kGtThreads, 1) gate_bwd_tma_kernel(const float *__restrict__ dh_out, const float *__restrict__ h,
-                                                                     const uint8_t *__restrict__ h_img_src, const uint2 *__restrict__ gates_packed,
-                                                                     const int32_t *__restrict__ indptr, const float *__restrict__ ds_in,
-                                                                     const int32_t *__restrict__ indptr_t, const int32_t *__restrict__ indices_t,
-                                                                     int32_t N, uint8_t *__restrict__ q_img, size_t img_stride,
-                                                                     float *__restrict__ dhz, float *__restrict__ db_fold, float *__restrict__ db_ih,
-                                                                     float *__restrict__ db_hh, int hints) {
-  extern __shared__ __align__(1024) uint8_t smem[];
-  const uint32_t sbase = smem_u32(smem);
-  const uint32_t bar0 = sbase + kGtOffBar;
-  auto full = [&](int i) { return bar0 + 8u * i; };
-  auto empty = [&](int i) { return bar0 + 8u * (kGtStages + i); };
-  const int lane = threadIdx.x & 31, warp = threadIdx.x >> 5;
-  const int64_t Npad = ((int64_t)N + kTileM - 1) / kTileM * kTileM;
-  const int num_blocks = (int)(Npad / kGtRows);
-  const int my_blocks = (num_blocks > (int)blockIdx.x) ? (num_blocks - 1 - (int)blockIdx.x) / (int)gridDim.x + 1 : 0;
-  if (threadIdx.x == 0) {
-    for (int i = 0; i < kGtStages; ++i) { mbar_init(full(i), 1); mbar_init(empty(i), kGtConsumers); }
-    mbar_fence_init();
-  }
-  __syncthreads();
-  pdl_launch_dependents();
-  pdl_wait();
-  float4 sum[7];
-#pragma unroll
-  for (int i = 0; i < 7; ++i) sum[i] = make_float4(0.f, 0.f, 0.f, 0.f);
-
-  auto fill = [&](int k) {
-    const uint64_t pol_saved = l2_policy((hints & 2) ? 1 : 0), pol_dh = l2_policy((hints & 8) ? 1 : 0);
-    const int stage = k % kGtStages;
-    const int64_t r0 = (int64_t)(blockIdx.x + (int64_t)k * gridDim.x) * kGtRows;
-    const int valid = (int)max((int64_t)0, min((int64_t)kGtRows, (int64_t)N - r0));
-    const uint32_t dst = sbase + stage * kGtStageBytes;
-    const uint32_t bytes = (uint32_t)valid * (kD * 4 + kD * 8) + (HF32 ? (uint32_t)valid * kD * 4 : (uint32_t)kGtRows * kD * 4);
-    mbar_arrive_expect_tx(full(stage), bytes);
-    if (valid > 0) {
-      bulk_g2s_hint(dst + kGtOffD, dh_out + r0 * kD, (uint32_t)valid * kD * 4, full(stage), pol_dh);
-      bulk_g2s_hint(dst + kGtOffG, gates_packed + r0 * kD, (uint32_t)valid * kD * 8, full(stage), pol_saved);
-    }
-    if (HF32) {
-      if (valid > 0) bulk_g2s_hint(dst + kGtOffH, h + r0 * kD, (uint32_t)valid * kD * 4, full(stage), pol_saved);
-    } else {
-      const uint8_t *tile = h_img_src + (size_t)(r0 >> 7) * kImageTileBytes + (size_t)(r0 & 127) * 128;
-#pragma unroll
-      for (int ch = 0; ch < 4; ++ch) bulk_g2s_hint(dst + kGtOffH + ch * (kGtRows * 128), tile + (size_t)ch * kChunkBytes, kGtRows * 128, full(stage), pol_saved);
-    }
-  };
-  if (warp == 0 && elect_one())
-    for (int k = 0; k < kGtStages && k < my_blocks; ++k) fill(k);
-  __syncwarp();
-  {
-    const int col = lane * 4;
-    const uint64_t pol_tmp = l2_policy((hints & 4) ? 2 : 0);
-    static_assert(kGtPre == 2, "lane slots below assume two prefetched neighbours per row");
-    auto load_scalars = [&](int kk) -> int {
-      int v = 0;
-      if (kk < my_blocks && lane < 8) {
-        const int64_t nd = (int64_t)(blockIdx.x + (int64_t)kk * gridDim.x) * kGtRows + warp + 16 * ((lane >> 1) & 1);
-        const int32_t *base = lane < 4 ? indptr : indptr_t;
-        if (nd < N && base) v = __ldcg(base + nd + (lane & 1));
-      }
-      return v;
-    };
-    auto load_ids = [&](int sc) -> int {
-      const int r_ = (lane >> 1) & 1, q_ = lane & 1;
-      const int tb_ = __shfl_sync(0xffffffffu, sc, 4 + 2 * r_), te_ = __shfl_sync(0xffffffffu, sc, 5 + 2 * r_);
-      int v = -1;
-      if (lane >= 8 && lane < 12 && tb_ + q_ < te_) v = __ldcg(indices_t + tb_ + q_);
-      return v;
-    };
-    int sc_cur = 0, sc_next = 0, id_cur = -1;
-    if constexpr (CSRP) {
-      sc_cur = load_scalars(0); sc_next = load_scalars(1);
-      id_cur = load_ids(sc_cur);
-    }
-    for (int k = 0; k < my_blocks; ++k) {
-      const int stage = k % kGtStages, use = k / kGtStages;
-      const int64_t r0 = (int64_t)(blockIdx.x + (int64_t)k * gridDim.x) * kGtRows;
-      int64_t node[2];
-      bool ok[2];
-      int tb[2], te[2], ip0[2], ip1[2];
-      int id[2][kGtPre];
-      if constexpr (CSRP) {
-        const int sc_next2 = load_scalars(k + 2);
-        const int id_next = load_ids(sc_next);
-#pragma unroll
-        for (int r = 0; r < 2; ++r) {
-          node[r] = r0 + warp + 16 * r;
-          ok[r] = node[r] < N;
-          ip0[r] = __shfl_sync(0xffffffffu, sc_cur, 2 * r); ip1[r] = __shfl_sync(0xffffffffu, sc_cur, 2 * r + 1);
-          tb[r] = __shfl_sync(0xffffffffu, sc_cur, 4 + 2 * r); te[r] = __shfl_sync(0xffffffffu, sc_cur, 5 + 2 * r);
-#pragma unroll
-          for (int q = 0; q < kGtPre; ++q) id[r][q] = __shfl_sync(0xffffffffu, id_cur, 8 + 2 * r + q);
-        }
-        sc_cur = sc_next; sc_next = sc_next2; id_cur = id_next;
-      } else {
-#pragma unroll
-        for (int r = 0; r < 2; ++r) {
-          node[r] = r0 + warp + 16 * r;
-          ok[r] = node[r] < N;
-          tb[r] = te[r] = ip0[r] = ip1[r] = 0;
-          if (ok[r]) {
-            ip0[r] = __ldcg(indptr + node[r]); ip1[r] = __ldcg(indptr + node[r] + 1);
-            if (indptr_t) { tb[r] = __ldcg(indptr_t + node[r]); te[r] = __ldcg(indptr_t + node[r] + 1); }
-          }
-        }
-#pragma unroll
-        for (int r = 0; r < 2; ++r)
-#pragma unroll
-          for (int q = 0; q < kGtPre; ++q) id[r][q] = (tb[r] + q < te[r]) ? __ldcg(indices_t + tb[r] + q) : -1;
-      }
-      float4 gv[2][kGtPre];
-#pragma unroll
-      for (int r = 0; r < 2; ++r)
-#pragma unroll
-        for (int q = 0; q < kGtPre; ++q) gv[r][q] = id[r][q] >= 0 ? ldg_cg_f4(ds_in + (size_t)id[r][q] * kD + col) : make_float4(0.f, 0.f, 0.f, 0.f);
-      mbar_wait(full(stage), use & 1);
-      const uint8_t *st = smem + stage * kGtStageBytes;
-#pragma unroll
-      for (int r = 0; r < 2; ++r) {
-        const int row = warp + 16 * r;
-        float4 d = make_float4(0.f, 0.f, 0.f, 0.f), hv = d, rr = d, zz = d, nn = d, gh = d;
-        if (ok[r]) {
-          d = *reinterpret_cast<const float4 *>(st + kGtOffD + row * (kD * 4) + col * 4);
-          const uint4 g0 = *reinterpret_cast<const uint4 *>(st + kGtOffG + row * (kD * 8) + col * 8);
-          const uint4 g1 = *reinterpret_cast<const uint4 *>(st + kGtOffG + row * (kD * 8) + col * 8 + 16);
-          unpack_gates(make_uint2(g0.x, g0.y), rr.x, zz.x, nn.x, gh.x);
-          unpack_gates(make_uint2(g0.z, g0.w), rr.y, zz.y, nn.y, gh.y);
-          unpack_gates(make_uint2(g1.x, g1.y), rr.z, zz.z, nn.z, gh.z);
-          unpack_gates(make_uint2(g1.z, g1.w), rr.w, zz.w, nn.w, gh.w);
-          if (HF32) {
-            hv = *reinterpret_cast<const float4 *>(st + kGtOffH + row * (kD * 4) + col * 4);
-          } else {
-            const uint32_t off = (uint32_t)((col >> 6) * (kGtRows * 128) + row * 128 + (((((col & 63) >> 3) ^ (row & 7)) & 7) << 4) + (col & 7) * 2);
-            const uint2 hh = *reinterpret_cast<const uint2 *>(st + kGtOffH + off);
-            const uint2 hl = *reinterpret_cast<const uint2 *>(st + kGtOffH + 2 * (kGtRows * 128) + off);
-            const float4 a = bf16x4_to_f4(hh), b = bf16x4_to_f4(hl);
-            hv = make_float4(a.x + b.x, a.y + b.y, a.z + b.z, a.w + b.w);
-          }
-#pragma unroll
-          for (int q = 0; q < kGtPre; ++q) f4_add(d, gv[r][q]);
-          for (int j = tb[r] + kGtPre; j < te[r]; ++j) f4_add(d, ldg_cg_f4(ds_in + (size_t)__ldcg(indices_t + j) * kD + col));
-        }
-        float4 qr = make_float4(0.f, 0.f, 0.f, 0.f), qz = qr, qn = qr, qnr = qr;
-        if (ok[r]) {
-          const float deg = (float)(ip1[r] - ip0[r]);
-          st_f4_hint(dhz + (size_t)node[r] * kD + col, make_float4(d.x * zz.x, d.y * zz.y, d.z * zz.z, d.w * zz.w), pol_tmp);
-#define BWDQ2(f)                                         \
-  {                                                      \
-    const float dz_ = d.f * (hv.f - nn.f);               \
-    const float dn_ = d.f * (1.f - zz.f);                \
-    qn.f = dn_ * (1.f - nn.f * nn.f);                    \
-    qz.f = dz_ * zz.f * (1.f - zz.f);                    \
-    qr.f = qn.f * gh.f * rr.f * (1.f - rr.f);            \
-    qnr.f = qn.f * rr.f;                                 \
-  }
-          BWDQ2(x) BWDQ2(y) BWDQ2(z) BWDQ2(w)
-#undef BWDQ2
-          f4_add(sum[0], qr); f4_add(sum[1], qz); f4_add(sum[2], qn); f4_add(sum[3], qnr);
-          f4_fma(sum[4], deg, qr); f4_fma(sum[5], deg, qz); f4_fma(sum[6], deg, qn);
-        }
-        if (node[r] < Npad) {
-          const size_t o_hi = image_offset(node[r], col, 0), o_lo = image_offset(node[r], col, 1);
-          uint2 ph, pl;
-          split4(qr, ph, pl);  *reinterpret_cast<uint2 *>(q_img + 0 * img_stride + o_hi) = ph; *reinterpret_cast<uint2 *>(q_img + 0 * img_stride + o_lo) = pl;
-          split4(qz, ph, pl);  *reinterpret_cast<uint2 *>(q_img + 1 * img_stride + o_hi) = ph; *reinterpret_cast<uint2 *>(q_img + 1 * img_stride + o_lo) = pl;
-          split4(qn, ph, pl);  *reinterpret_cast<uint2 *>(q_img + 2 * img_stride + o_hi) = ph; *reinterpret_cast<uint2 *>(q_img + 2 * img_stride + o_lo) = pl;
-          split4(qnr, ph, pl); *reinterpret_cast<uint2 *>(q_img + 3 * img_stride + o_hi) = ph; *reinterpret_cast<uint2 *>(q_img + 3 * img_stride + o_lo) = pl;
-        }
-      }
-      __syncwarp();
-      if (lane == 0) mbar_arrive(empty(stage));
-      if (warp == 0 && k + kGtStages < my_blocks) {
-        if (elect_one()) {
-          mbar_wait(empty(stage), use & 1);
-          fill(k + kGtStages);
-        }
-        __syncwarp();
-      }
-    }
-  }
-  __syncthreads();
-  float *red = reinterpret_cast<float *>(smem);
-  {
-#pragma unroll
-    for (int i = 0; i < 7; ++i) *reinterpret_cast<float4 *>(&red[(warp * 7 + i) * kD + lane * 4]) = sum[i];
-  }
-  __syncthreads();
-  for (int i = threadIdx.x; i < 7 * kD; i += kGtThreads) {
-    float v_ = 0.f;
-#pragma unroll
-    for (int w = 0; w < kGtConsumers; ++w) v_ += red[(w * 7) * kD + i];
     const int which = i >> 7, c_ = i & 127;
     if (which == 0) { atomicAdd(db_ih + c_, v_); atomicAdd(db_hh + c_, v_); }
     else if (which == 1) { atomicAdd(db_ih + kD + c_, v_); atomicAdd(db_hh + kD + c_, v_); }
@@ -511,6 +304,324 @@
   }
 }
 
+constexpr int kGtRows = 32;
+constexpr int kGtOffD = 0, kGtOffG = kGtRows * kD * 4, kGtOffH = kGtOffG + kGtRows * kD * 8;
+static_assert(kGtOffH + kGtRows * kD * 4 == kD3StageBytes, "phase A's operands fill exactly one stage");
+static_assert(4 * kGtRows == kTileM, "four CTAs per tile");
+constexpr int kGtPre = 2;
+constexpr int kGtRowsPerWarp = kGtRows / kEpiWarps;
+
+__device__ __forceinline__ void fence_proxy_async_global() { asm volatile("fence.proxy.async.global;" ::: "memory"); }
+__device__ __forceinline__ void cluster_arrive_release() { asm volatile("barrier.cluster.arrive.release;" ::: "memory"); }
+__device__ __forceinline__ void cluster_wait_acquire() { asm volatile("barrier.cluster.wait.acquire;" ::: "memory"); }
+
+template <bool HF32, bool CSRP>
+__global__ void __launch_bounds__(kD3Threads, 1) bwd_step_fused_kernel(const float *__restrict__ dh_out, const float *__restrict__ h,
+                                                                       const uint8_t *__restrict__ h_img_src, const uint2 *__restrict__ gates_packed,
+                                                                       const int32_t *__restrict__ indptr, const float *__restrict__ ds_in,
+                                                                       const int32_t *__restrict__ indptr_t, const int32_t *__restrict__ indices_t,
+                                                                       int32_t N, uint8_t *__restrict__ q_img, size_t img_stride,
+                                                                       const uint8_t *__restrict__ packed3, float *__restrict__ ds, float *__restrict__ dh,
+                                                                       float *__restrict__ db_fold, float *__restrict__ db_ih, float *__restrict__ db_hh,
+                                                                       int hints) {
+  extern __shared__ uint8_t smem_raw[];
+  uint8_t *smem = reinterpret_cast<uint8_t *>((reinterpret_cast<uintptr_t>(smem_raw) + 1023) & ~(uintptr_t)1023);
+  const uint32_t sbase = smem_u32(smem);
+  const uint32_t bar0 = sbase + kD3OffBar;
+  auto full = [&](int i) { return bar0 + 8u * i; };
+  auto empty = [&](int i) { return bar0 + 8u * (kD3Stages + i); };
+  const uint32_t w_full = bar0 + 8u * (2 * kD3Stages);
+  const int tron = (g_trace_on == 1);
+
+  const int warp = threadIdx.x >> 5, lane = threadIdx.x & 31;
+  const int rh = blockIdx.x & 3, role = rh >> 1, half = rh & 1;
+  const int cluster = blockIdx.x >> 2, num_clusters = gridDim.x >> 2;
+  const int num_tiles = (N + kTileM - 1) / kTileM;
+  const int my_tiles = (num_tiles > cluster) ? (num_tiles - 1 - cluster) / num_clusters + 1 : 0;
+  const int tile0 = num_tiles - 1 - cluster;
+  auto tile_of = [&](int k) { return tile0 - k * num_clusters; };
+
+  if (threadIdx.x == 0) {
+    for (int i = 0; i < kD3Stages; ++i) { mbar_init(full(i), 1); mbar_init(empty(i), kEpiWarps); }
+    mbar_init(w_full, 1);
+    mbar_fence_init();
+  }
+  __syncthreads();
+  if (threadIdx.x == 0) trace_stamp(tron, 0, 0);
+  pdl_launch_dependents();
+
+  if (warp == kEpiWarps) {
+    const uint64_t pol_saved = l2_policy((hints & 2) ? 1 : 0), pol_dh = l2_policy((hints & 8) ? 1 : 0);
+    const uint64_t pol_q = l2_policy((hints & 64) ? 1 : 0);
+    if (my_tiles > 0 && elect_one()) {
+      mbar_arrive_expect_tx(w_full, kD3WBytes);
+      bulk_g2s(sbase, packed3 + (size_t)rh * kD3WBytes, kD3WBytes, w_full);
+    }
+    __syncwarp();
+    pdl_wait();
+    int cc = 0;
+    for (int k = 0; k < my_tiles; ++k, cc += 4) {
+      const int tile = tile_of(k);
+      if (elect_one()) {
+        const int stage = cc % kD3Stages, use = cc / kD3Stages;
+        if (use > 0) mbar_wait_bounded(empty(stage), (use - 1) & 1);
+        const int64_t r0 = (int64_t)tile * kTileM + kGtRows * rh;
+        const int valid = (int)max((int64_t)0, min((int64_t)kGtRows, (int64_t)N - r0));
+        const uint32_t dst = sbase + kD3OffStage + stage * kD3StageBytes;
+        const uint32_t bytes = (uint32_t)valid * (kD * 4 + kD * 8) + (HF32 ? (uint32_t)valid * kD * 4 : (uint32_t)kGtRows * kD * 4);
+        mbar_arrive_expect_tx(full(stage), bytes);
+        if (valid > 0) {
+          bulk_g2s_hint(dst + kGtOffD, dh_out + r0 * kD, (uint32_t)valid * kD * 4, full(stage), pol_dh);
+          bulk_g2s_hint(dst + kGtOffG, gates_packed + r0 * kD, (uint32_t)valid * kD * 8, full(stage), pol_saved);
+        }
+        if (HF32) {
+          if (valid > 0) bulk_g2s_hint(dst + kGtOffH, h + r0 * kD, (uint32_t)valid * kD * 4, full(stage), pol_saved);
+        } else {
+          const uint8_t *t0 = h_img_src + (size_t)tile * kImageTileBytes + (size_t)(kGtRows * rh) * 128;
+#pragma unroll
+          for (int ch = 0; ch < 4; ++ch) bulk_g2s_hint(dst + kGtOffH + ch * (kGtRows * 128), t0 + (size_t)ch * kChunkBytes, kGtRows * 128, full(stage), pol_saved);
+        }
+      }
+      __syncwarp();
+      cluster_arrive_release();
+      cluster_wait_acquire();
+      if (elect_one()) {
+        fence_proxy_async_global();
+        for (int g = 0; g < 3; ++g) {
+          const int m = g < 2 ? g : (role == 0 ? 2 : 3);
+          const int c = cc + 1 + g, stage = c % kD3Stages, use = c / kD3Stages;
+          if (use > 0) mbar_wait_bounded(empty(stage), (use - 1) & 1);
+          mbar_arrive_expect_tx(full(stage), kD3StageBytes);
+          bulk_g2s_hint(sbase + kD3OffStage + stage * kD3StageBytes, q_img + (size_t)m * img_stride + (size_t)tile * kImageTileBytes,
+                        kD3StageBytes, full(stage), pol_q);
+          if (g != 1) trace_stamp(tron, k, g == 0 ? 1 : 2);
+        }
+      }
+      __syncwarp();
+    }
+  } else {
+    pdl_wait();
+    const int col = lane * 4;
+#define DDFA_POL_TMP l2_policy((hints & 4) ? 2 : 0)
+#define DDFA_POL_DHZ l2_policy((hints & 8) ? 1 : 0)
+    const int wg = warp >> 2;
+    const int row0 = wg * 64 + (warp & 3) * 16 + (lane >> 2);
+    const int col0 = half * 64 + 2 * (lane & 3);
+    const bool tr = (warp == 0 && lane == 0);
+    float4 sum[7];
+#pragma unroll
+    for (int i = 0; i < 7; ++i) sum[i] = make_float4(0.f, 0.f, 0.f, 0.f);
+    static_assert(kGtPre == 2 && kGtRowsPerWarp == 4, "lane slots below assume four rows per warp and two prefetched neighbours per row");
+    auto node_of = [&](int tile, int r) { return (int64_t)tile * kTileM + kGtRows * rh + warp + kEpiWarps * r; };
+    auto load_scalars = [&](int kk) -> int {
+      int v = 0;
+      if (kk < my_tiles && lane < 16) {
+        const int64_t nd = node_of(tile_of(kk), (lane >> 1) & 3);
+        const int32_t *base = lane < 8 ? indptr : indptr_t;
+        if (nd < N && base) v = __ldcg(base + nd + (lane & 1));
+      }
+      return v;
+    };
+    auto load_ids = [&](int sc) -> int {
+      const int r_ = (lane >> 1) & 3, q_ = lane & 1;
+      const int tb_ = __shfl_sync(0xffffffffu, sc, 8 + 2 * r_), te_ = __shfl_sync(0xffffffffu, sc, 9 + 2 * r_);
+      int v = -1;
+      if (lane >= 16 && lane < 24 && tb_ + q_ < te_) v = __ldcg(indices_t + tb_ + q_);
+      return v;
+    };
+    int sc_cur = 0, sc_next = 0, id_cur = -1;
+    if constexpr (CSRP) {
+      sc_cur = load_scalars(0); sc_next = load_scalars(1);
+      id_cur = load_ids(sc_cur);
+    }
+    int cc = 0;
+    for (int k = 0; k < my_tiles; ++k) {
+      const int tile = tile_of(k);
+      {
+        const int stage = cc % kD3Stages, use = cc / kD3Stages;
+        ++cc;
+        const int64_t node0 = node_of(tile, 0);
+        bool ok[kGtRowsPerWarp];
+        int tb[kGtRowsPerWarp], te[kGtRowsPerWarp];
+        float deg[kGtRowsPerWarp];
+        int id[kGtRowsPerWarp][kGtPre];
+        if constexpr (CSRP) {
+          const int sc_next2 = load_scalars(k + 2);
+          const int id_next = load_ids(sc_next);
+#pragma unroll
+          for (int r = 0; r < kGtRowsPerWarp; ++r) {
+            ok[r] = node0 + kEpiWarps * r < N;
+            deg[r] = (float)(__shfl_sync(0xffffffffu, sc_cur, 2 * r + 1) - __shfl_sync(0xffffffffu, sc_cur, 2 * r));
+            tb[r] = __shfl_sync(0xffffffffu, sc_cur, 8 + 2 * r); te[r] = __shfl_sync(0xffffffffu, sc_cur, 9 + 2 * r);
+#pragma unroll
+            for (int q = 0; q < kGtPre; ++q) id[r][q] = __shfl_sync(0xffffffffu, id_cur, 16 + 2 * r + q);
+          }
+          sc_cur = sc_next; sc_next = sc_next2; id_cur = id_next;
+        } else {
+#pragma unroll
+          for (int r = 0; r < kGtRowsPerWarp; ++r) {
+            const int64_t nd = node0 + kEpiWarps * r;
+            ok[r] = nd < N;
+            tb[r] = te[r] = 0;
+            deg[r] = 0.f;
+            if (ok[r]) {
+              deg[r] = (float)(__ldcg(indptr + nd + 1) - __ldcg(indptr + nd));
+              if (indptr_t) { tb[r] = __ldcg(indptr_t + nd); te[r] = __ldcg(indptr_t + nd + 1); }
+            }
+          }
+#pragma unroll
+          for (int r = 0; r < kGtRowsPerWarp; ++r)
+#pragma unroll
+            for (int q = 0; q < kGtPre; ++q) id[r][q] = (tb[r] + q < te[r]) ? __ldcg(indices_t + tb[r] + q) : -1;
+        }
+        float4 gv[kGtRowsPerWarp][kGtPre];
+#pragma unroll
+        for (int r = 0; r < kGtRowsPerWarp; ++r)
+#pragma unroll
+          for (int q = 0; q < kGtPre; ++q) gv[r][q] = id[r][q] >= 0 ? ldg_cg_f4(ds_in + (size_t)id[r][q] * kD + col) : make_float4(0.f, 0.f, 0.f, 0.f);
+        mbar_wait_bounded(full(stage), use & 1);
+        const uint8_t *st = smem + kD3OffStage + stage * kD3StageBytes;
+#pragma unroll
+        for (int r = 0; r < kGtRowsPerWarp; ++r) {
+          const int row = warp + kEpiWarps * r;
+          float4 d = make_float4(0.f, 0.f, 0.f, 0.f), hv = d, rr = d, zz = d, nn = d, gh = d;
+          if (ok[r]) {
+            d = *reinterpret_cast<const float4 *>(st + kGtOffD + row * (kD * 4) + col * 4);
+            const uint4 g0 = *reinterpret_cast<const uint4 *>(st + kGtOffG + row * (kD * 8) + col * 8);
+            const uint4 g1 = *reinterpret_cast<const uint4 *>(st + kGtOffG + row * (kD * 8) + col * 8 + 16);
+            unpack_gates(make_uint2(g0.x, g0.y), rr.x, zz.x, nn.x, gh.x);
+            unpack_gates(make_uint2(g0.z, g0.w), rr.y, zz.y, nn.y, gh.y);
+            unpack_gates(make_uint2(g1.x, g1.y), rr.z, zz.z, nn.z, gh.z);
+            unpack_gates(make_uint2(g1.z, g1.w), rr.w, zz.w, nn.w, gh.w);
+            if (HF32) {
+              hv = *reinterpret_cast<const float4 *>(st + kGtOffH + row * (kD * 4) + col * 4);
+            } else {
+              const uint32_t off = (uint32_t)((col >> 6) * (kGtRows * 128) + row * 128 + (((((col & 63) >> 3) ^ (row & 7)) & 7) << 4) + (col & 7) * 2);
+              const uint2 hh = *reinterpret_cast<const uint2 *>(st + kGtOffH + off);
+              const uint2 hl = *reinterpret_cast<const uint2 *>(st + kGtOffH + 2 * (kGtRows * 128) + off);
+              const float4 a = bf16x4_to_f4(hh), b = bf16x4_to_f4(hl);
+              hv = make_float4(a.x + b.x, a.y + b.y, a.z + b.z, a.w + b.w);
+            }
+#pragma unroll
+            for (int q = 0; q < kGtPre; ++q) f4_add(d, gv[r][q]);
+            for (int j = tb[r] + kGtPre; j < te[r]; ++j) f4_add(d, ldg_cg_f4(ds_in + (size_t)__ldcg(indices_t + j) * kD + col));
+          }
+          float4 qr = make_float4(0.f, 0.f, 0.f, 0.f), qz = qr, qn = qr, qnr = qr;
+          const int64_t node = node0 + kEpiWarps * r;
+          if (ok[r]) {
+            st_f4_hint(dh + (size_t)node * kD + col, make_float4(d.x * zz.x, d.y * zz.y, d.z * zz.z, d.w * zz.w), DDFA_POL_TMP);
+#define BWDQ2(f)                                         \
+  {                                                      \
+    const float dz_ = d.f * (hv.f - nn.f);               \
+    const float dn_ = d.f * (1.f - zz.f);                \
+    qn.f = dn_ * (1.f - nn.f * nn.f);                    \
+    qz.f = dz_ * zz.f * (1.f - zz.f);                    \
+    qr.f = qn.f * gh.f * rr.f * (1.f - rr.f);            \
+    qnr.f = qn.f * rr.f;                                 \
+  }
+            BWDQ2(x) BWDQ2(y) BWDQ2(z) BWDQ2(w)
+#undef BWDQ2
+            f4_add(sum[0], qr); f4_add(sum[1], qz); f4_add(sum[2], qn); f4_add(sum[3], qnr);
+            f4_fma(sum[4], deg[r], qr); f4_fma(sum[5], deg[r], qz); f4_fma(sum[6], deg[r], qn);
+          }
+          const size_t o_hi = image_offset(node, col, 0), o_lo = image_offset(node, col, 1);
+          uint2 ph, pl;
+          split4(qr, ph, pl);  *reinterpret_cast<uint2 *>(q_img + 0 * img_stride + o_hi) = ph; *reinterpret_cast<uint2 *>(q_img + 0 * img_stride + o_lo) = pl;
+          split4(qz, ph, pl);  *reinterpret_cast<uint2 *>(q_img + 1 * img_stride + o_hi) = ph; *reinterpret_cast<uint2 *>(q_img + 1 * img_stride + o_lo) = pl;
+          split4(qn, ph, pl);  *reinterpret_cast<uint2 *>(q_img + 2 * img_stride + o_hi) = ph; *reinterpret_cast<uint2 *>(q_img + 2 * img_stride + o_lo) = pl;
+          split4(qnr, ph, pl); *reinterpret_cast<uint2 *>(q_img + 3 * img_stride + o_hi) = ph; *reinterpret_cast<uint2 *>(q_img + 3 * img_stride + o_lo) = pl;
+        }
+        __syncwarp();
+        if (lane == 0) mbar_arrive(empty(stage));
+      }
+      fence_proxy_async_global();
+      cluster_arrive_release();
+      cluster_wait_acquire();
+      if (tr) trace_stamp(tron, k, 11);
+      if (k == 0) mbar_wait_bounded(w_full, 0);
+      float acc[32];
+      int pending = -1;
+      if (tr) { trace_stamp(tron, k, 7); trace_stamp(tron, k, 3); }
+      for (int g = 0; g < 3; ++g, ++cc) {
+        const int stage = cc % kD3Stages, use = cc / kD3Stages;
+        mbar_wait_bounded(full(stage), use & 1);
+        if (tr && g != 1) trace_stamp(tron, k, g == 0 ? 4 : 5);
+        wgmma_fence();
+        const uint32_t a0 = sbase + kD3OffStage + stage * kD3StageBytes + wg * 8192;
+        const uint32_t w0 = sbase + g * 4 * kD3WChunkBytes;
+#pragma unroll
+        for (int kb = 0; kb < 2; ++kb) {
+#pragma unroll
+          for (int k4 = 0; k4 < 4; ++k4) {
+            const uint64_t a_hi = gmma_desc(a0 + kb * kChunkBytes + k4 * 32), a_lo = gmma_desc(a0 + (2 + kb) * kChunkBytes + k4 * 32);
+            const uint64_t b_hi = gmma_desc(w0 + kb * kD3WChunkBytes + k4 * 32), b_lo = gmma_desc(w0 + (2 + kb) * kD3WChunkBytes + k4 * 32);
+            wgmma_n64<0, 0>(acc, a_hi, b_hi, (g == 0 && kb == 0 && k4 == 0) ? 0u : 1u);
+            wgmma_n64<0, 0>(acc, a_hi, b_lo, 1u);
+            wgmma_n64<0, 0>(acc, a_lo, b_hi, 1u);
+          }
+        }
+        wgmma_commit();
+        wgmma_wait<1>();
+        __syncwarp();
+        if (pending >= 0 && lane == 0) mbar_arrive(empty(pending));
+        pending = stage;
+      }
+      float2 dv[8];
+      auto fetch_dv = [&](int hh) {
+        const uint64_t pol_dhz = DDFA_POL_DHZ;
+        const int64_t node = (int64_t)tile * kTileM + row0 + 8 * hh;
+#pragma unroll
+        for (int j = 0; j < 8; ++j) {
+          dv[j] = make_float2(0.f, 0.f);
+          if (role == 1 && node < N) {
+            const float *p = dh + node * kD + col0 + 8 * j;
+            dv[j] = make_float2(ldg_cg_f32_hint(p, pol_dhz), ldg_cg_f32_hint(p + 1, pol_dhz));
+          }
+        }
+      };
+      fetch_dv(0);
+      wgmma_wait<0>();
+      wgmma_fence_regs(acc);
+      if (tr) { trace_stamp(tron, k, 6); trace_stamp(tron, k, 8); }
+      __syncwarp();
+      if (lane == 0) mbar_arrive(empty(pending));
+      if (tr) trace_stamp(tron, k, 9);
+#pragma unroll
+      for (int hh = 0; hh < 2; ++hh) {
+        if (hh == 1) fetch_dv(1);
+        const int64_t node = (int64_t)tile * kTileM + row0 + 8 * hh;
+        if (node < N) {
+          const uint64_t pol_tmp = DDFA_POL_TMP;
+          float *out = role == 0 ? ds : dh;
+#pragma unroll
+          for (int j = 0; j < 8; ++j)
+            st_f2_hint(out + node * kD + col0 + 8 * j, make_float2(acc[4 * j + 2 * hh] + dv[j].x, acc[4 * j + 2 * hh + 1] + dv[j].y), pol_tmp);
+        }
+      }
+      if (tr) trace_stamp(tron, k, 10);
+    }
+#undef DDFA_POL_TMP
+#undef DDFA_POL_DHZ
+    asm volatile("bar.sync 1, %0;" ::"n"(32 * kEpiWarps) : "memory");
+    float *red = reinterpret_cast<float *>(smem + kD3OffStage);
+#pragma unroll
+    for (int i = 0; i < 7; ++i) *reinterpret_cast<float4 *>(&red[(warp * 7 + i) * kD + col]) = sum[i];
+  }
+  __syncthreads();
+  const float *red = reinterpret_cast<const float *>(smem + kD3OffStage);
+  for (int i = threadIdx.x; i < 7 * kD; i += kD3Threads) {
+    float v_ = 0.f;
+#pragma unroll
+    for (int w = 0; w < kEpiWarps; ++w) v_ += red[(w * 7) * kD + i];
+    const int which = i >> 7, c_ = i & 127;
+    if (which == 0) { atomicAdd(db_ih + c_, v_); atomicAdd(db_hh + c_, v_); }
+    else if (which == 1) { atomicAdd(db_ih + kD + c_, v_); atomicAdd(db_hh + kD + c_, v_); }
+    else if (which == 2) atomicAdd(db_ih + 2 * kD + c_, v_);
+    else if (which == 3) atomicAdd(db_hh + 2 * kD + c_, v_);
+    else atomicAdd(db_fold + (which - 4) * kD + c_, v_);
+  }
+}
+
 constexpr int kWgSlotBytes = kImageTileBytes;
 constexpr int kWgSlots = 3;
 constexpr int kWgOffBar = kWgSlots * kWgSlotBytes;
@@ -678,6 +789,51 @@
   return DDFA_OK;
 }
 
+template <bool HF32, bool CSRP>
+static int bwd_fused_max_clusters(int *out) {
+  static std::atomic<int> cached{0};
+  int v = cached.load(std::memory_order_relaxed);
+  if (v == 0) {
+    DDFA_CUDA(cudaFuncSetAttribute(tc2b::bwd_step_fused_kernel<HF32, CSRP>, cudaFuncAttributeMaxDynamicSharedMemorySize, tc2b::kD3SmemAlloc));
+    cudaLaunchConfig_t cfg = {};
+    cfg.gridDim = dim3(kNumSMs / 4 * 4);
+    cfg.blockDim = dim3(tc2b::kD3Threads);
+    cfg.dynamicSmemBytes = tc2b::kD3SmemAlloc;
+    cudaLaunchAttribute attr;
+    attr.id = cudaLaunchAttributeClusterDimension;
+    attr.val.clusterDim.x = 4;
+    attr.val.clusterDim.y = 1;
+    attr.val.clusterDim.z = 1;
+    cfg.attrs = &attr;
+    cfg.numAttrs = 1;
+    DDFA_CUDA(cudaOccupancyMaxActiveClusters(&v, tc2b::bwd_step_fused_kernel<HF32, CSRP>, &cfg));
+    if (v < 1) {
+      set_error("tcgen05 engine (bwd): bwd_step_fused_kernel fits no 4-CTA cluster on this device");
+      return DDFA_ERR_CUDA;
+    }
+    cached.store(v, std::memory_order_relaxed);
+  }
+  *out = v;
+  return DDFA_OK;
+}
+int gru_tc2b_fused_max_clusters(int *out) { return bwd_fused_max_clusters<false, true>(out); }
+
+template <bool HF32, bool CSRP>
+static int launch_bwd_fused(int tiles, cudaStream_t stream, const float *dh_out, const float *h, const void *h_img_in, const void *gates_packed,
+                            const int32_t *indptr, const float *ds_in, const int32_t *indptr_t, const int32_t *indices_t, int32_t N,
+                            uint8_t *q_img, size_t img, const uint8_t *packed, float *ds, float *dh, float *db_fold, float *db_ih, float *db_hh) {
+  int clusters = 0;
+  const int rc = bwd_fused_max_clusters<HF32, CSRP>(&clusters);
+  if (rc != DDFA_OK) return rc;
+  if (clusters > tiles) clusters = tiles;
+  DDFA_CUDA(cudaFuncSetAttribute(tc2b::bwd_step_fused_kernel<HF32, CSRP>, cudaFuncAttributeMaxDynamicSharedMemorySize, tc2b::kD3SmemAlloc));
+  DDFA_CUDA(launch_chain_cluster(4, 4, tc2b::bwd_step_fused_kernel<HF32, CSRP>, dim3(clusters * 4), dim3(tc2b::kD3Threads), tc2b::kD3SmemAlloc,
+                                 stream, dh_out, h, static_cast<const uint8_t *>(h_img_in), static_cast<const uint2 *>(gates_packed), indptr,
+                                 ds_in, ds_in ? indptr_t : nullptr, indices_t, N, q_img, img, packed, ds, dh, db_fold, db_ih, db_hh, l2_hints()));
+  DDFA_CHECK_LAUNCH("tc2b::bwd_step_fused_kernel");
+  return DDFA_OK;
+}
+
 int gru_tc2_step_bwd(const float *dh_out, const float *ds_in, const int32_t *indptr_t, const int32_t *indices_t, const float *h,
                      const void *h_img_in, const void *s_img, const float *gates, const void *gates_packed, const int32_t *indptr, int32_t N, float *ds, float *dh, float *dw_fold, float *db_fold, float *db_ih,
                      float *dw_hh, float *db_hh, void *workspace, size_t workspace_bytes, int wgrad_mode, cudaStream_t stream) {
@@ -693,39 +849,28 @@
   uint8_t *packed = static_cast<uint8_t *>(workspace);
   const size_t img = tcc::image_bytes(N);
   uint8_t *h_img_ws = packed + kPackedTotal;
-  float *dhz = reinterpret_cast<float *>(h_img_ws + img);
   float *partial = reinterpret_cast<float *>(h_img_ws + 3 * img);
   uint8_t *q_img = packed + bwd_fixed_bytes(N) + (size_t)q_slot * 4 * img;
   const uint8_t *h_img = h_img_in ? static_cast<const uint8_t *>(h_img_in) : h_img_ws;
-  const int64_t rows = ((int64_t)N + tcc::kTileM - 1) / tcc::kTileM * tcc::kTileM;
-  unsigned gb_grid = 1;
-  {
+  const int tiles = (N + tcc::kTileM - 1) / tcc::kTileM;
+  if (gates_packed && gate_bwd_tma()) {
+    const bool csrp = gate_bwd_tma() >= 2;
+    int rc = DDFA_OK;
+    if (h) rc = csrp ? launch_bwd_fused<true, true>(tiles, stream, dh_out, h, h_img_in, gates_packed, indptr, ds_in, indptr_t, indices_t, N, q_img, img, packed, ds, dh, db_fold, db_ih, db_hh)
+                     : launch_bwd_fused<true, false>(tiles, stream, dh_out, h, h_img_in, gates_packed, indptr, ds_in, indptr_t, indices_t, N, q_img, img, packed, ds, dh, db_fold, db_ih, db_hh);
+    else   rc = csrp ? launch_bwd_fused<false, true>(tiles, stream, dh_out, h, h_img_in, gates_packed, indptr, ds_in, indptr_t, indices_t, N, q_img, img, packed, ds, dh, db_fold, db_ih, db_hh)
+                     : launch_bwd_fused<false, false>(tiles, stream, dh_out, h, h_img_in, gates_packed, indptr, ds_in, indptr_t, indices_t, N, q_img, img, packed, ds, dh, db_fold, db_ih, db_hh);
+    if (rc != DDFA_OK) return rc;
+  } else {
+    const int64_t rows = (int64_t)tiles * tcc::kTileM;
     const int64_t want = (rows + tc2b::kGbWarps - 1) / tc2b::kGbWarps;
-    gb_grid = (unsigned)(want < 2 * kNumSMs ? want : 2 * kNumSMs);
-  }
-  if (gates_packed && gate_bwd_tma()) {
-    const int blocks32 = (int)(rows / tc2b::kGtRows);
-    const int grid = blocks32 < kNumSMs ? blocks32 : kNumSMs;
-    const bool csrp = gate_bwd_tma() >= 2;
-#define DDFA_GT_LAUNCH(HF32, CSRP)                                                                                                             \
-  do {                                                                                                                                         \
-    DDFA_CUDA(cudaFuncSetAttribute(tc2b::gate_bwd_tma_kernel<HF32, CSRP>, cudaFuncAttributeMaxDynamicSharedMemorySize, tc2b::kGtSmem));        \
-    DDFA_CUDA(launch_chain(4, tc2b::gate_bwd_tma_kernel<HF32, CSRP>, dim3(grid), dim3(tc2b::kGtThreads), tc2b::kGtSmem, stream, dh_out, h,     \
-                           static_cast<const uint8_t *>(h_img_in), static_cast<const uint2 *>(gates_packed), indptr, ds_in,                    \
-                           ds_in ? indptr_t : nullptr, indices_t, N, q_img, img, dhz, db_fold, db_ih, db_hh, l2_hints()));                    \
-  } while (0)
-    if (h) { if (csrp) DDFA_GT_LAUNCH(true, true); else DDFA_GT_LAUNCH(true, false); }
-    else   { if (csrp) DDFA_GT_LAUNCH(false, true); else DDFA_GT_LAUNCH(false, false); }
-#undef DDFA_GT_LAUNCH
-  } else
-  DDFA_CUDA(launch_chain(4, tc2b::gate_bwd_image_kernel, dim3(gb_grid), dim3(32 * tc2b::kGbWarps), 0, stream, dh_out, h,
-                         static_cast<const uint8_t *>(h_img_in), gates, static_cast<const uint4 *>(gates_packed), indptr, ds_in,
-                         ds_in ? indptr_t : nullptr, indices_t, N, q_img, img, h_img_in ? nullptr : h_img_ws, dhz, db_fold, db_ih, db_hh,
-                         l2_hints()));
-  DDFA_CHECK_LAUNCH("tc2b::gate_bwd_image_kernel");
-  DDFA_CUDA(cudaFuncSetAttribute(tc2b::wgrad_kernel, cudaFuncAttributeMaxDynamicSharedMemorySize, tc2b::kWgSmemAlloc));
-  const int tiles = (N + tcc::kTileM - 1) / tcc::kTileM;
-  {
+    const unsigned gb_grid = (unsigned)(want < 2 * kNumSMs ? want : 2 * kNumSMs);
+    float *dhz = reinterpret_cast<float *>(h_img_ws + img);
+    DDFA_CUDA(launch_chain(4, tc2b::gate_bwd_image_kernel, dim3(gb_grid), dim3(32 * tc2b::kGbWarps), 0, stream, dh_out, h,
+                           static_cast<const uint8_t *>(h_img_in), gates, static_cast<const uint4 *>(gates_packed), indptr, ds_in,
+                           ds_in ? indptr_t : nullptr, indices_t, N, q_img, img, h_img_in ? nullptr : h_img_ws, dhz, db_fold, db_ih, db_hh,
+                           l2_hints()));
+    DDFA_CHECK_LAUNCH("tc2b::gate_bwd_image_kernel");
     DDFA_CUDA(cudaFuncSetAttribute(tc2b::dgrad3_kernel, cudaFuncAttributeMaxDynamicSharedMemorySize, tc2b::kD3SmemAlloc));
     int groups = kNumSMs / 4;
     if (groups > tiles) groups = tiles;
@@ -733,6 +878,7 @@
                            static_cast<const uint8_t *>(packed), N, ds, dh, l2_hints()));
     DDFA_CHECK_LAUNCH("tc2b::dgrad3_kernel");
   }
+  DDFA_CUDA(cudaFuncSetAttribute(tc2b::wgrad_kernel, cudaFuncAttributeMaxDynamicSharedMemorySize, tc2b::kWgSmemAlloc));
   if (wgrad_mode >= 16) return DDFA_OK;
   tc2b::WgBatch one = {};
   one.s_img[0] = static_cast<const uint8_t *>(s_img);
```

Result: faster. 94520, median of 6 (+5.4%).
